# facebookresearch/unbiased-teacher-v2

Hardware: AMD Instinct MI355X
Metric: images/sec/node (labeled+unlabeled) UTv2 step, R50-FPN 1333x800 (higher is better)
Workload: dtype f16

## Files before the change

### include/utv2.h

```cpp
#ifndef UTV2_H
#define UTV2_H
#include <stdint.h>
#ifdef __cplusplus
extern "C" {
#endif

typedef struct ihipStream_t* utv2_stream_t;

int utv2_conv2d_nhwc_fwd(const float* x, const float* w, float* y, const float* scale, const float* bias,
                         const float* residual, int N, int H, int W, int C, int K, int KH, int KW, int stride, int pad,
                         int in_dil, int OH, int OW, int relu, int accumulate, int Kred, utv2_stream_t stream);
int utv2_conv2d_stem_fwd(const float* x, const float* w, void* y, int y_dtype, const float* scale, const float* bias, int N,
                         int H, int W, int K, int KH, int KW, int stride, int pad, int OH, int OW, int relu, int Kred,
                         utv2_stream_t stream);
int utv2_conv2d_wgrad_splits(int N, int OH, int OW, int K, int Kred);
int64_t utv2_conv2d_wgrad_workspace_floats(int N, int OH, int OW, int K, int Kred);
int utv2_conv2d_nhwc_wgrad(const float* x, const float* dy, float* dw, float* ws, int N, int H, int W, int C, int K,
                           int KH, int KW, int stride, int pad, int OH, int OW, int accumulate, utv2_stream_t stream);
int utv2_colsum(const float* g, float* db, float* ws, int M, int C, int accumulate, utv2_stream_t stream);
int utv2_weight_flip_transpose(const float* w, float* wt, int K, int KH, int KW, int C, utv2_stream_t stream);

int utv2_conv2d_ml_fwd(const float* x, const float* w, float* y, const float* scale, const float* bias,
                       const float* residual, int nlev, const int* H_host, const int* W_host, int N, int C, int K, int KH,
                       int KW, int pad, int relu, int accumulate, utv2_stream_t stream);
int utv2_conv2d_ml_wgrad(const float* x, const float* dy, float* dw, float* ws, int nlev, const int* H_host,
                         const int* W_host, int N, int C, int K, int KH, int KW, int pad, int accumulate,
                         utv2_stream_t stream);

#define UTV2_F32 0
#define UTV2_BF16 1
int utv2_conv2d_bf16_supported(int C, int KH, int KW);

int utv2_conv_clock_probe(double* ghz, double* lifetime_us);
int utv2_conv2d_nhwc_fwd_bf16_bits(const void* x, int x_dtype, const void* w16, void* y, int y_dtype, const float* scale,
                                   const float* bias, const void* residual, const void* mask, const void* post_mask, int N, int H, int W,
                                   int C, int K, int KH, int KW, int stride, int pad, int in_dil, int OH, int OW, int relu, int accumulate,
                                   const int* rowinfo, void* relu_bits, const void* mask_bits, const void* post_mask_bits,
                                   utv2_stream_t stream);
int utv2_conv2d_ml_fwd_bf16_g(const void* x, int x_dtype, int x_pitch, const void* w16, void* y, int y_dtype, int y_pitch,
                              const float* scale, const float* bias, const void* residual, int nlev, const int* H_host,
                              const int* W_host, int N, int C, int K, int KH, int KW, int pad, int relu, int accumulate, int groups,
                              float* gn_part, const int* rowinfo, utv2_stream_t stream);
int utv2_conv2d_ml_fwd_bf16_gnb(const void* x, int x_pitch, const void* w16, void* y, int nlev, const int* H_host, const int* W_host, int N,
                                int C, int K, int KH, int KW, int pad, int groups, const int* rowinfo, const void* mask_bits,
                                const void* gnb_x, float* gnb_part, utv2_stream_t stream);
int utv2_conv2d_wgrad_bf16_splits(int M, int K, int Kred);
int64_t utv2_conv2d_wgrad_bf16_workspace_floats(int M, int K, int Kred);
int utv2_conv2d_wgrad_bf16_g(const void* x, int x_dtype, int x_pitch, const void* dy, int dy_dtype, int dy_pitch, float* dw, float* db,
                             float* ws, const int* rowinfo, const float* rowscale, int M, int C, int K, int KH, int KW, int accumulate,
                             int groups, utv2_stream_t stream);
int utv2_conv2d_wgrad_bf16_d(const void* x, int x_dtype, int x_pitch, const void* dy, int dy_dtype, int dy_pitch, float* dw, float* db,
                             float* ws, const int* rowinfo, const float* rowscale, int M, int C, int K, int KH, int KW, int accumulate,
                             int groups, void* pending, utv2_stream_t stream);
int64_t utv2_wgrad_fold_table_bytes(void);
int utv2_wgrad_fold_pending(const void* pending);
int utv2_wgrad_fold_flush(void* pending, utv2_stream_t stream);
int utv2_conv2d_stem_fwd_bf16(const void* xpad16, const void* w16s, void* y, int y_dtype, const float* scale,
                              const float* bias, int N, int H, int W, int K, int OH, int OW, int relu, utv2_stream_t stream);
int utv2_rowinfo_nhwc(int* out, int N, int H, int W, int OH, int OW, int stride, int pad, int KH, int KW, int64_t start,
                      utv2_stream_t stream);
int utv2_f32_to_bf16(const float* src, void* dst16, int64_t n, utv2_stream_t stream);
int utv2_weight_flip_transpose_bf16(const float* w, void* wt16, const float* scale, int K, int KH, int KW, int C,
                                    utv2_stream_t stream);
int utv2_pad_cols_bf16(const void* src, int src_dtype, void* dst16, int64_t rows, int c, int cpad, utv2_stream_t stream);
int utv2_weight_flip_transpose_bf16_batched(const float* arena, const float* scales, void* bank, const void* table, int nlayers,
                                            utv2_stream_t stream);

int utv2_ema_axpby(float* teacher, const float* student, int64_t n, double keep_rate, utv2_stream_t stream);
int utv2_sgd_momentum(float* param, float* grad, float* mom_buf, int64_t n, float lr, float momentum, float weight_decay,
                      float grad_scale, int zero_grad, utv2_stream_t stream);
int utv2_amp_found_inf(const float* grad, int64_t n, float* state, utv2_stream_t stream);
int utv2_sgd_momentum_amp(float* param, const float* grad, float* mom_buf, int64_t n, float lr, float momentum, float weight_decay,
                          float grad_scale, const float* state, utv2_stream_t stream);
int utv2_amp_update_scale(float* state, float growth_factor, float backoff_factor, int growth_interval, utv2_stream_t stream);
int utv2_ema_axpby_m16(float* teacher, const float* student, void* mirror16, int64_t n, double keep_rate, utv2_stream_t stream);
int utv2_sgd_momentum_m16(float* param, float* grad, float* mom_buf, void* mirror16, int64_t n, float lr, float momentum, float weight_decay,
                          float grad_scale, int zero_grad, utv2_stream_t stream);
int utv2_sgd_momentum_amp_m16(float* param, const float* grad, float* mom_buf, void* mirror16, int64_t n, float lr, float momentum,
                              float weight_decay, float grad_scale, const float* state, utv2_stream_t stream);

int utv2_relu_bwd_scale(const void* dy, const void* y, const float* scale, void* out, int64_t M, int C, int dtype,
                        utv2_stream_t stream);
int utv2_add(const float* a, const float* b, float* out, int64_t n, utv2_stream_t stream);
int utv2_maxpool3x3s2_nhwc(const void* x, int x_dtype, void* y, int y_dtype, int N, int H, int W, int C, int OH, int OW,
                           utv2_stream_t stream);
int utv2_maxpool3x3s2_bwd_nhwc(const void* x, int x_dtype, const void* dpool, void* dx, int g_dtype, int N, int H, int W, int C, int OH,
                               int OW, int relu, utv2_stream_t stream);
int utv2_upsample2x_add_nhwc(const void* lateral, const void* top, void* out, int N, int H, int W, int C, int dtype,
                             utv2_stream_t stream);
int utv2_downsample2x_sum_nhwc(const void* g, void* dtop, int N, int TH, int TW, int C, int accumulate, int dtype,
                               utv2_stream_t stream);
int utv2_zero_interleave2x_nhwc(const void* src, const void* mask, void* dst, int N, int H, int W, int C, int dtype, utv2_stream_t stream);
int utv2_zero_interleave2x_add_nhwc(const void* src, const void* mask, const void* mask_bits, const void* add, void* dst, int N, int H, int W,
                                    int C, utv2_stream_t stream);
int utv2_preprocess_image(const void* src, int is_u8, float* dst, int H, int W, int Hp, int Wp,
                          const float* mean3_host, const float* std3_host, utv2_stream_t stream);
int utv2_preprocess_image_bf16pad(const void* src, int is_u8, void* dst16, int H, int W, int Hp, int Wp,
                                  const float* mean3_host, const float* std3_host, utv2_stream_t stream);
int utv2_preprocess_images_bf16pad(const void* const* src_host, int is_u8, void* dst16, const int* H_host, const int* W_host, int N,
                                   int Hp, int Wp, const float* mean3_host, const float* std3_host, utv2_stream_t stream);
int utv2_frozenbn_fold(const float* w, const float* b, const float* mean, const float* var, float* scale, float* shift,
                       int n, float eps, utv2_stream_t stream);
int64_t utv2_groupnorm_seg_workspace_floats(int nseg, const int* seg_rows_host, int C);
int utv2_groupnorm_relu_seg_fwd(const void* x, const float* gamma, const float* beta, void* y, float* mean, float* rstd,
                                float* ws, int nseg, const int* seg_rows_host, int C, int G, float eps, int relu, int dtype,
                                utv2_stream_t stream);
int utv2_groupnorm_relu_seg_fwd_p32(const void* x, const float* gamma, const float* beta, void* y, float* mean, float* rstd,
                                    const float* part32, int nseg, const int* seg_rows_host, int C, int G, float eps, int relu,
                                    utv2_stream_t stream);
int utv2_groupnorm_relu_seg_fwd_p32b(const void* x, const float* gamma, const float* beta, void* y, float* mean, float* rstd,
                                     const float* part32, int nseg, const int* seg_rows_host, int C, int G, float eps, int relu,
                                     void* relu_bits, utv2_stream_t stream);
int utv2_groupnorm_relu_seg_bwd(const void* dy, const void* y, const void* x, const float* mean, const float* rstd,
                                const float* gamma, const float* beta, void* dx, float* dgamma, float* dbeta, float* ws,
                                int nseg, const int* seg_rows_host, int C, int G, int relu, int dtype, utv2_stream_t stream);
int64_t utv2_groupnorm_seg_chunks(int nseg, const int* seg_rows_host);
int utv2_groupnorm_relu_seg_bwd_colsum(const void* dy, const void* y, const void* x, const float* mean, const float* rstd,
                                       const float* gamma, const float* beta, void* dx, float* dgamma, float* dbeta, float* ws,
                                       int nseg, const int* seg_rows_host, int C, int G, int relu, int dtype, float* colsum_part,
                                       utv2_stream_t stream);
int utv2_groupnorm_seg_bwd_p64(const void* g, const void* x, const float* mean, const float* rstd, const float* gamma, void* dx,
                               float* dgamma, float* dbeta, float* ws, int nseg, const int* seg_rows_host, int C, int G,
                               const float* part64, float* colsum_part, utv2_stream_t stream);
int utv2_colsum_partials(const float* partial, float* db, int nb, int K, int accumulate, utv2_stream_t stream);
int64_t utv2_groupnorm_workspace_floats(int N, int HW, int C);
int utv2_groupnorm_relu_fwd(const float* x, const float* gamma, const float* beta, float* y, float* mean, float* rstd,
                            float* ws, int N, int HW, int C, int G, float eps, int relu, utv2_stream_t stream);
int utv2_groupnorm_relu_bwd(const float* dy, const float* y, const float* x, const float* mean, const float* rstd,
                            const float* gamma, float* dx, float* dgamma, float* dbeta, float* ws, int N, int HW, int C,
                            int G, int relu, utv2_stream_t stream);

int utv2_fcos_targets(int num_levels, const int* H_host, const int* W_host, const int* strides_host,
                      const float* soi_host, int N, int MAXG, const float* gt_boxes, const int* gt_classes,
                      const unsigned char* gt_valid, const float* gt_std, int num_classes, int drop_empty,
                      float center_radius, const unsigned char* img_active, int* labels, float* reg_targets, float* bvars,
                      int* gt_inds, utv2_stream_t stream);
int utv2_fcos_targets_range(int num_levels, const int* H_host, const int* W_host, const int* strides_host, const float* soi_host, int N,
                            int MAXG, const float* gt_boxes, const int* gt_classes, const unsigned char* gt_valid, const float* gt_std,
                            int gt_img0, int gt_imgs, int num_classes, int drop_empty, float center_radius,
                            const unsigned char* img_active, int* labels, float* reg_targets, float* bvars, int* gt_inds,
                            utv2_stream_t stream);
int utv2_sigmoid_focal_fwd(const float* logits, const int* labels, int64_t P, int C, float alpha, float gamma,
                           float* loss_sum, float* ws, utv2_stream_t stream);
int utv2_sigmoid_focal_bwd(const float* logits, const int* labels, int64_t P, int C, float alpha, float gamma,
                           const float* coef, float* dlogits, utv2_stream_t stream);
int utv2_fcos_loc_terms_fwd(const int* labels, const float* box, int box_stride, const float* reg_targets,
                            const float* bvars, int64_t P, int num_classes, int reg_max, float ts_better, float ts_cert,
                            int flags, float* sums, float* ws, utv2_stream_t stream);
int utv2_fcos_loc_terms_bwd(const int* labels, const float* box, int box_stride, const float* reg_targets,
                            const float* bvars, int64_t P, int num_classes, int reg_max, float ts_better, float ts_cert,
                            int flags, const float* coef, float* dbox, utv2_stream_t stream);
int utv2_sigmoid_focal_bwd_acc(const float* logits, const int* labels, int64_t P, int C, float alpha, float gamma, const float* coef,
                               const float* gscale, float* dlogits, int accumulate, utv2_stream_t stream);
int utv2_fcos_loc_terms_bwd_acc(const int* labels, const float* box, int box_stride, const float* reg_targets, const float* bvars,
                                int64_t P, int num_classes, int reg_max, float ts_better, float ts_cert, int flags, const float* coef8,
                                const float* gscale, float* dbox, int accumulate, utv2_stream_t stream);
int utv2_fcos_loss_combine(const float* focal_sup, const float* sums_sup, const float* focal_cls, const float* sums_cls,
                           const float* sums_reg, const float* norm, float world, int flags, float kl_weight, const float* wmul_host,
                           const float* wdiv_host, float* rec, float* coef, utv2_stream_t stream);
int utv2_fcos_rank_keys(const float* logits, const float* box, int box_stride, int reg_max, int N, int HW, int C,
                        float thr, int method, long long* keys, int64_t key_row_stride, utv2_stream_t stream);
int64_t utv2_topk_rows_workspace_bytes(int rows, int k);
int utv2_topk_rows_i64(const long long* keys, const long long* row_off, int rows, int64_t max_width, int k, long long* out,
                       void* ws, utv2_stream_t stream);
int utv2_fcos_decode(const long long* topkeys, int K, const float* logits, const float* box, int box_stride, int reg_max,
                     int N, int HW, int Wl, int C, int stride, int level, int method, int MAXC, int slot0, float* oboxes,
                     float* oscores, int* ocls, float* oloc, float* octr, float* oconf, float* ostd, int* olevel,
                     unsigned char* ovalid, utv2_stream_t stream);
int utv2_fcos_loc_terms_cont_fwd(const int* labels, const float* box, int box_stride, const float* reg_targets, const float* bvars,
                                 int64_t P, int num_classes, float ts_better, float ts_cert, int flags, float* sums, float* ws,
                                 utv2_stream_t stream);
int utv2_fcos_loc_terms_cont_bwd(const int* labels, const float* box, int box_stride, const float* reg_targets, const float* bvars,
                                 int64_t P, int num_classes, float ts_better, float ts_cert, int flags, const float* coef, float* dbox,
                                 utv2_stream_t stream);
int utv2_fcos_loc_terms_cont_bwd_acc(const int* labels, const float* box, int box_stride, const float* reg_targets, const float* bvars,
                                     int64_t P, int num_classes, float ts_better, float ts_cert, int flags, const float* coef8,
                                     const float* gscale, float* dbox, int accumulate, utv2_stream_t stream);
int utv2_fcos_decode_cont(const long long* topkeys, int K, const float* logits, const float* box, int box_stride, int N, int HW, int Wl,
                          int C, int stride, int level, int method, int MAXC, int slot0, float* oboxes, float* oscores, int* ocls,
                          float* oloc, float* octr, float* oconf, float* ostd, int* olevel, unsigned char* ovalid,
                          utv2_stream_t stream);
int utv2_scale_cols(float* y, int64_t rows, int row_stride, int ncols, const float* s, utv2_stream_t stream);
int utv2_scale_cols_bwd(float* g, const float* ypost, int64_t rows, int row_stride, int ncols, const float* s, float* dsum,
                        float* ws, utv2_stream_t stream);
int utv2_scale_cols_ml(float* y, int nlev, const int64_t* row0_host, int row_stride, int ncols, const float* const* s_host,
                       utv2_stream_t stream);
int utv2_scale_cols_bwd_ml(float* g, const float* ypost, int nlev, const int64_t* row0_host, int row_stride, int ncols,
                           const float* const* s_host, float* const* sgrad_host, float* ws, utv2_stream_t stream);
int utv2_scale_cols_bwd_ml_pad16(const float* g, const float* ypost, int nlev, const int64_t* row0_host, int row_stride, int ncols,
                                 const float* const* s_host, float* const* sgrad_host, float* ws, void* out16, int cpad, utv2_stream_t stream);

int utv2_nms_mpad(int M);
int64_t utv2_nms_workspace_bytes(int N, int M);
int utv2_nms_batched(const float* boxes, const float* scores, const int* cls, const unsigned char* valid, int N, int M,
                     float iou_thr, int class_aware, int post_topk, int max_out, int* keep, int* keep_count, void* ws,
                     utv2_stream_t stream);
int utv2_box_iou(const float* a, const float* b, int A, int B, float* out, utv2_stream_t stream);

int utv2_match_boxes(const float* boxes, int64_t box_img_stride, int N, int P, const float* gt_boxes,
                     const unsigned char* gt_valid, int G, float* max_iou, int* arg, unsigned* gt_max_bits,
                     utv2_stream_t stream);
int utv2_match_lowq(const float* boxes, int64_t box_img_stride, int N, int P, const float* gt_boxes,
                    const unsigned char* gt_valid, int G, const unsigned* gt_max_bits, unsigned char* lowq,
                    utv2_stream_t stream);
#define UTV2_POOLER_ALIGN_V2 0
#define UTV2_POOLER_ALIGN 1
#define UTV2_POOLER_MAX 2
int utv2_roi_pooler_fwd(int pooler, int sampling_ratio, int num_levels, int min_level, const void* const* feats_host,
                        const int* H_host, const int* W_host, const float* scales_host, const float* rois, const int* roi_batch,
                        const unsigned char* roi_valid, int R, int C, int PH, int PW, void* out, int* argmax, int dtype,
                        utv2_stream_t stream);
int utv2_roi_pooler_bwd(int pooler, int sampling_ratio, int num_levels, int min_level, float* const* dfeats_host, const int* H_host,
                        const int* W_host, const float* scales_host, const float* rois, const int* roi_batch,
                        const unsigned char* roi_valid, int R, int C, int PH, int PW, const void* dy, const int* argmax, int dtype,
                        utv2_stream_t stream);
int utv2_roi_pooler_bwd_tiled(int pooler, int sampling_ratio, int num_levels, int min_level, void* const* dfeats_host,
                              const int* H_host, const int* W_host, const float* scales_host, const float* rois,
                              const unsigned char* roi_valid, int N, int rois_per_image, int C, int PH, int PW, const void* dy,
                              const int* argmax, int dy_dtype, int out_dtype, utv2_stream_t stream);
int utv2_rpn_rank_keys(const float* head, int num_levels, const int* hw_host, int N, int A, int ch, int64_t* keys, utv2_stream_t stream);
int utv2_rpn_decode(const int64_t* top, int maxk, const float* head, const float* anchors, const float* image_hw, int num_levels,
                    const int* hw_host, const int* k_host, int N, int A, int ch, const float* weights_host, float scale_clamp,
                    float min_size, float* boxes, float* scores, int* lvls, unsigned char* keep, utv2_stream_t stream);
int utv2_nms_pack(const int* kidx, const int* cnt, const float* boxes, const float* scores, int N, int M, int D, float* oboxes, float* oscores,
                  unsigned char* ovalid, utv2_stream_t stream);
int utv2_roi_infer_keys(const float* probs, const float* deltas, const float* prop, const unsigned char* valid, const float* whwh, int N, int P,
                        int K, int nbox, float wx, float wy, float scale_clamp, float thr, float* boxes, int64_t* keys, utv2_stream_t stream);
int utv2_roi_infer_gather(const int64_t* top, const float* boxes, int N, int P, int K, int nbox, int k, float thr, float* sc, int64_t* rows,
                          int* cls, float* cb, unsigned char* valid, utv2_stream_t stream);
int utv2_roi_infer_pack(const int* kidx, const int* cnt, const float* cb, const float* sc, const int* cls, const int64_t* rows, const float* stdl,
                        int N, int P, int k, int D, int nbox, float* oboxes, float* oscores, int* ocls, float* ostd, int64_t* orows,
                        unsigned char* ovalid, utv2_stream_t stream);
int utv2_rpn_loss_fwd(const float* obj, const float* deltas, int head, int num_levels, const int* hw_host, int N, int A, int ch, int R,
                      const float* anchors, const int64_t* pos_idx, const unsigned char* pos_valid, int npos, const int64_t* neg_idx,
                      const unsigned char* neg_valid, int nneg, const int* matched, const unsigned char* has_gt, const float* gt_boxes,
                      const float* gt_scores, int G, const float* weights_host, float* sums, float* gobj, float* gdl, utv2_stream_t stream);
int utv2_rpn_loss_bwd(const float* gobj, const float* gdl, const float* gout_cls, const float* gout_loc, int head, int num_levels,
                      const int* hw_host, int N, int A, int ch, int R, const int64_t* pos_idx, const unsigned char* pos_valid, int npos,
                      const int64_t* neg_idx, const unsigned char* neg_valid, int nneg, float* grad_obj, float* grad_deltas,
                      utv2_stream_t stream);
int utv2_rpn_loss_fwd_range(const float* obj, const float* deltas, int head, int num_levels, const int* hw_host, int N, int batch, int img0,
                            int A, int ch, int R, const float* anchors, const int64_t* pos_idx, const unsigned char* pos_valid, int npos,
                            const int64_t* neg_idx, const unsigned char* neg_valid, int nneg, const int* matched,
                            const unsigned char* has_gt, const float* gt_boxes, const float* gt_scores, int G, const float* weights_host,
                            float* sums, float* gobj, float* gdl, utv2_stream_t stream);
int utv2_rpn_loss_bwd_range(const float* gobj, const float* gdl, const float* gout_cls, const float* gout_loc, int head, int num_levels,
                            const int* hw_host, int N, int batch, int img0, int A, int ch, int R, const int64_t* pos_idx,
                            const unsigned char* pos_valid, int npos, const int64_t* neg_idx, const unsigned char* neg_valid, int nneg,
                            float* grad_obj, float* grad_deltas, utv2_stream_t stream);
int utv2_rpn_sample_keys(const float* max_iou, const unsigned char* lowq, const unsigned char* gt_valid, int G, const float* keys, int N,
                         int R, float lo, float hi, int64_t* out, utv2_stream_t stream);
int utv2_rpn_sample_unpack(const int64_t* top, int k, int N, int npos_max, int nneg_max, const unsigned char* gt_valid, int G,
                           int64_t* pos_idx, unsigned char* pos_valid, int64_t* neg_idx, unsigned char* neg_valid, unsigned char* has_gt,
                           utv2_stream_t stream);
int utv2_roi_sample(const float* boxes, const unsigned char* valid, const float* max_iou, const int* argmax, const float* keys, int N, int P,
                    const float* gt_boxes, const int* gt_classes, const unsigned char* gt_valid, const float* gt_scores, const float* gt_std,
                    int G, float iou_thr, int num_classes, int batch, int nfg_max, float* out_boxes, int64_t* out_classes,
                    float* out_gt_boxes, unsigned char* out_valid, int64_t* out_idx, float* out_conf, float* out_std, utv2_stream_t stream);
int utv2_roi_box_loss(const float* deltas, const float* stdl, int64_t ld, const int64_t* cls, const float* prop, const float* gtb,
                      const float* gstd, int R, int num_classes, int nbox, int mode, float wx, float wy, float scale_clamp, float ts_better,
                      float t_cert, float* sum, float* gdeltas, float* gstd_out, utv2_stream_t stream);
int utv2_softmax_focal_fwd(const float* logits, const int* target, int R, int C, float gamma, float* loss_sum, float* ws,
                           utv2_stream_t stream);
int utv2_softmax_focal_bwd(const float* logits, const int* target, int R, int C, float gamma, const float* coef,
                           float* dlogits, utv2_stream_t stream);
int utv2_rcnn_loss_combine(const float* rpn_sup, const float* rpn_uns, const float* focal_sup, const float* focal_uns, const float* box_sup,
                           const float* box_uns, const int* tgt_sup, int n_sup, const int* tgt_uns, int n_uns, float rpn_norm_sup,
                           float rpn_norm_uns, float w_rpn_cls, float w_rpn_loc, float w_box, const float* wt_host, float* rec, float* coef,
                           utv2_stream_t stream);

int utv2_stem_pool_fwd_bf16(const void* xpad16, const void* w16s, void* y, const float* scale, const float* shift, int N, int H, int W,
                            int K, utv2_stream_t stream);

int utv2_bottleneck_supported(int C, int MID, int has_shortcut);
int utv2_bottleneck_fwd_bf16(const void* x, void* y, const void* w1, const void* w2, const void* w3, const void* wsc, const float* s1,
                             const float* b1, const float* s2, const float* b2, const float* s3, const float* b3, const float* ssc,
                             const float* bsc, int N, int H, int W, int C, int MID, utv2_stream_t stream);

int64_t utv2_aug_resize_workspace_bytes(int H, int W, int OH, int OW);
int utv2_aug_resize_bilinear_u8(const unsigned char* src, int H, int W, unsigned char* dst, int OH, int OW, int flip, void* ws,
                                utv2_stream_t stream);
int utv2_aug_gray_mean_u8(const unsigned char* img, int64_t npix, void* sum_ws, int* mean_out, utv2_stream_t stream);
int utv2_aug_blend_u8(unsigned char* img, int64_t npix, int mode, float alpha, const int* mean, utv2_stream_t stream);
int utv2_aug_hue_u8(unsigned char* img, int64_t npix, int shift, utv2_stream_t stream);
int utv2_aug_grayscale_u8(unsigned char* img, int64_t npix, utv2_stream_t stream);
int utv2_aug_box_blur_u8(const unsigned char* src, unsigned char* dst, int H, int W, int vertical, int radius, int ww, int fw,
                         utv2_stream_t stream);
int utv2_aug_erase_u8(unsigned char* img, int H, int W, int i, int j, int h, int w, const float* noise, utv2_stream_t stream);
int utv2_aug_hwc_to_chw_u8(const unsigned char* src, unsigned char* dst, int64_t npix, utv2_stream_t stream);

int utv2_coco_pair_keys(const float* scores, const int* cls, const long long* off, int N, int K, long long* keys, utv2_stream_t stream);
int utv2_coco_seg_offsets(const long long* keys, int64_t n, int64_t nseg, long long* off, utv2_stream_t stream);
int utv2_coco_rank_keys(const long long* key1, const long long* pair_off, int64_t D, int K, int max_dets, long long* key2,
                        unsigned char* rank, utv2_stream_t stream);
int64_t utv2_coco_eval_workspace_bytes(int64_t D, int K);
int utv2_coco_match(const float* dbox, const long long* dperm, const long long* dpair_off, const double* gbox, const unsigned char* gcrowd,
                    const double* garea, const long long* gperm, const long long* gpair_off, int N, int K, int64_t D, int max_dets,
                    int max_gt, const double* iou_thrs_host, const double* area_rng_host, void* ws, utv2_stream_t stream);
int utv2_coco_accumulate(const long long* perm2, const long long* cat_off, const unsigned char* rank, int K, int64_t D,
                         const double* rec_thrs_host, const void* ws, double* precision, double* recall, utv2_stream_t stream);

int utv2_gconv3x3_supported(int C, int G);
int utv2_gconv3x3_fwd(const void* x, const void* w, int op_dtype, void* y, int y_dtype, const float* scale, const float* shift, int N,
                      int H, int W, int C, int G, int stride, int OH, int OW, int relu, utv2_stream_t stream);
int utv2_gconv3x3_dgrad(const void* dy, const void* w, int op_dtype, void* dx, int dx_dtype, const float* scale, const void* mask,
                        const void* residual, int N, int H, int W, int C, int G, int stride, int OH, int OW, utv2_stream_t stream);
int utv2_gconv3x3_wgrad_splits(int N, int OH, int OW, int C, int G);
int64_t utv2_gconv3x3_wgrad_workspace_floats(int N, int OH, int OW, int C, int G);
int utv2_gconv3x3_wgrad(const void* x, const void* dy, int op_dtype, float* dw, float* ws, const float* scale, int N, int H, int W,
// ... 7 lines not shown
```

### unbiased-teacher-v2_amd/csrc/fcos.hip

```cpp
#include "common.h"

#define MAX_LEVELS 8

struct LevelTable {
  int num_levels;
  int H[MAX_LEVELS], W[MAX_LEVELS], stride[MAX_LEVELS];
  int off[MAX_LEVELS + 1];
  float soi_lo[MAX_LEVELS], soi_hi[MAX_LEVELS];
};

__device__ __forceinline__ int level_of(const LevelTable& t, int loc) {
  int l = 0;
#pragma unroll
  for (int i = 1; i < MAX_LEVELS; ++i)
    if (i < t.num_levels && loc >= t.off[i]) l = i;
  return l;
}

#define TG_MAXG 256
__global__ __launch_bounds__(256) void fcos_targets_kernel(LevelTable lt, int N, int MAXG, const float* __restrict__ gt_boxes,
                                                         const int* __restrict__ gt_classes,
                                                         const unsigned char* __restrict__ gt_valid,
                                                         const float* __restrict__ gt_std, int num_classes, int drop_empty,
                                                         float center_radius, const unsigned char* __restrict__ img_active,
// ... 19 lines not shown
  const int G = scount;
  for (int k = threadIdx.x; k < G; k += blockDim.x) {
    const float* b = gt_boxes + ((size_t)gi * MAXG + sidx[k]) * 4;
    sb[k][0] = b[0]; sb[k][1] = b[1]; sb[k][2] = b[2]; sb[k][3] = b[3];
    sarea[k] = (b[2] - b[0]) * (b[3] - b[1]);
  }
  __syncthreads();
  const int loc = blockIdx.x * blockDim.x + threadIdx.x;
  if (loc >= L) return;
  const int l = level_of(lt, loc);
  const int hw = loc - lt.off[l];
  const int HWl = lt.H[l] * lt.W[l];
  const int y = hw / lt.W[l], x = hw - y * lt.W[l];
  const float s = (float)lt.stride[l];
  const float xs = (float)(x * lt.stride[l]) + (float)(lt.stride[l] / 2);
  const float ys = (float)(y * lt.stride[l]) + (float)(lt.stride[l] / 2);
  const size_t p = (size_t)N * lt.off[l] + (size_t)n * HWl + hw;
  const bool inactive = !in_range || (img_active != nullptr && !img_active[n]);
  if (G == 0 || inactive) {
    labels[p] = ((drop_empty & 1) || inactive) ? -1 : num_classes;
    gt_inds[p] = -1;
#pragma unroll
    for (int e = 0; e < 4; ++e) { reg_targets[p * 4 + e] = 0.f; bvars[p * 4 + e] = 0.f; }
    return;
  }
  const float INF = 100000000.f;
  float best = INF;
  int bi = 0;
  const bool cs = center_radius > 0.f;
  const float sr = s * center_radius;
  const bool cs_none = cs && (sb[0][0] + sb[0][2]) * 0.5f * (float)L == 0.f;
  bool inside_any = false, sampled_any = false;
  for (int k = 0; k < G; ++k) {
    const float lft = xs - sb[k][0], top = ys - sb[k][1], rgt = sb[k][2] - xs, bot = sb[k][3] - ys;
    float mn = fminf(fminf(lft, top), fminf(rgt, bot));
    inside_any |= mn > 0.f;
    const float mx = fmaxf(fmaxf(lft, top), fmaxf(rgt, bot));
    if (cs) {
      const float cx = (sb[k][0] + sb[k][2]) * 0.5f, cy = (sb[k][1] + sb[k][3]) * 0.5f;
      const float xmin = cx - sr, ymin = cy - sr, xmax = cx + sr, ymax = cy + sr;
      const float x0 = xmin > sb[k][0] ? xmin : sb[k][0], y0 = ymin > sb[k][1] ? ymin : sb[k][1];
      const float x1 = xmax > sb[k][2] ? sb[k][2] : xmax, y1 = ymax > sb[k][3] ? sb[k][3] : ymax;
      mn = cs_none ? -1.f : fminf(fminf(xs - x0, ys - y0), fminf(x1 - xs, y1 - ys));
    }
    sampled_any |= mn > 0.f;
    float a = sarea[k];
    if (!(mn > 0.f)) a = INF;
    if (!(mx >= lt.soi_lo[l] && mx <= lt.soi_hi[l])) a = INF;
    if (a < best) { best = a; bi = k; }
  }
  const bool bg = (best == INF);
  const int g = sidx[bi];
  const bool ignored = (drop_empty & 2) && inside_any && !sampled_any;
  labels[p] = ignored ? -1 : bg ? num_classes : gt_classes[gi * MAXG + g];
  gt_inds[p] = g;
  reg_targets[p * 4 + 0] = (xs - sb[bi][0]) / s;
  reg_targets[p * 4 + 1] = (ys - sb[bi][1]) / s;
  reg_targets[p * 4 + 2] = (sb[bi][2] - xs) / s;
  reg_targets[p * 4 + 3] = (sb[bi][3] - ys) / s;
#pragma unroll
  for (int e = 0; e < 4; ++e) bvars[p * 4 + e] = bg ? 99999.0f : (gt_std ? gt_std[((size_t)gi * MAXG + g) * 4 + e] : 0.f);
}

__device__ __forceinline__ float focal_term(float x, float t, float alpha, float gamma, float* dldx) {
  const float e = expf(-fabsf(x));
  const float r = 1.f / (1.f + e);
  const float p = x >= 0.f ? r : e * r;
  const float l1p = log1pf(e);
  const float ce = fmaxf(x, 0.f) - x * t + l1p;
  const float q = x >= 0.f ? e * r : r;
  const float pt = p * t + q * (1.f - t);
  const float om = q * t + p * (1.f - t);
  const float mod = (gamma == 2.f) ? om * om : powf(om, gamma);
  const float at = alpha >= 0.f ? alpha * t + (1.f - alpha) * (1.f - t) : 1.f;
  if (dldx) {
    *dldx = at * (2.f * t - 1.f) * mod * (gamma * pt * (-ce) - om);
  }
  return ce * mod * at;
}

__global__ __launch_bounds__(256) void focal_fwd_kernel(const float* __restrict__ logits, const int* __restrict__ labels, size_t P,
                                                      int C, float alpha, float gamma, float* __restrict__ partial) {
  __shared__ float red[4];
  float acc = 0.f;
  if ((C & 3) == 0 && P * (size_t)C < (1ull << 32)) {
    const unsigned C4 = (unsigned)C >> 2, total4 = (unsigned)(P * (size_t)C4);
    for (unsigned i4 = blockIdx.x * blockDim.x + threadIdx.x; i4 < total4; i4 += gridDim.x * blockDim.x) {
      const unsigned row = i4 / C4;
      const int c = (int)(i4 - row * C4) * 4;
      const int lab = labels[row];
      if (lab < 0) continue;
      const f32x4 v = ((const f32x4*)logits)[i4];
#pragma unroll
      for (int e = 0; e < 4; ++e) acc += focal_term(v[e], lab == c + e ? 1.f : 0.f, alpha, gamma, nullptr);
    }
  } else {
    const size_t total = P * (size_t)C;
    const size_t stride = (size_t)gridDim.x * blockDim.x;
    for (size_t i = (size_t)blockIdx.x * blockDim.x + threadIdx.x; i < total; i += stride) {
      const size_t row = i / C;
      const int c = (int)(i - row * C);
      const int lab = labels[row];
      if (lab < 0) continue;
      acc += focal_term(logits[i], lab == c ? 1.f : 0.f, alpha, gamma, nullptr);
    }
  }
  const float s = block_reduce_sum(acc, red);
  if (threadIdx.x == 0) partial[blockIdx.x] = s;
}

__global__ __launch_bounds__(256) void focal_bwd_kernel(const float* __restrict__ logits, const int* __restrict__ labels, size_t P,
                                                      int C, float alpha, float gamma, const float* __restrict__ coef,
                                                      float* __restrict__ dlogits, const float* __restrict__ gscale, int accumulate) {
  const float k = coef[0] * (gscale ? gscale[0] : 1.f);
  if ((C & 3) == 0 && P * (size_t)C < (1ull << 32)) {
    const unsigned C4 = (unsigned)C >> 2, total4 = (unsigned)(P * (size_t)C4);
    for (unsigned i4 = blockIdx.x * blockDim.x + threadIdx.x; i4 < total4; i4 += gridDim.x * blockDim.x) {
      const unsigned row = i4 / C4;
      const int c = (int)(i4 - row * C4) * 4;
      const int lab = labels[row];
      if (accumulate && lab < 0) continue;
      f32x4 g = {0.f, 0.f, 0.f, 0.f};
      if (accumulate) g = ((const f32x4*)dlogits)[i4];
      if (lab >= 0) {
        const f32x4 v = ((const f32x4*)logits)[i4];
#pragma unroll
        for (int e = 0; e < 4; ++e) {
          float ge;
          focal_term(v[e], lab == c + e ? 1.f : 0.f, alpha, gamma, &ge);
          g[e] += ge * k;
        }
      }
      ((f32x4*)dlogits)[i4] = g;
    }
    return;
  }
  const size_t total = P * (size_t)C;
  size_t i = (size_t)blockIdx.x * blockDim.x + threadIdx.x;
  const size_t stride = (size_t)gridDim.x * blockDim.x;
  for (; i < total; i += stride) {
    const size_t row = i / C;
    const int c = (int)(i - row * C);
    const int lab = labels[row];
    if (accumulate && lab < 0) continue;
    float g = 0.f;
    if (lab >= 0) {
      focal_term(logits[i], lab == c ? 1.f : 0.f, alpha, gamma, &g);
      g *= k;
    }
    dlogits[i] = accumulate ? dlogits[i] + g : g;
  }
}

__global__ __launch_bounds__(256) void sum_partials_kernel(const float* __restrict__ partial, int n, int ncols,
                                                           float* __restrict__ out) {
  __shared__ double red[256];
  const int c = blockIdx.x;
  double s = 0.0;
  for (int r = threadIdx.x; r < n; r += 256) s += (double)partial[(size_t)r * ncols + c];
  red[threadIdx.x] = s;
  __syncthreads();
  for (int w = 128; w > 0; w >>= 1) {
    if (threadIdx.x < w) red[threadIdx.x] += red[threadIdx.x + w];
    __syncthreads();
  }
  if (threadIdx.x == 0) out[c] = (float)red[0];
}

#define LT_NSUM 8
struct LocTerms {
  float d[4];
  float ctr_t, iou, giou_l, nll;
};

template <int R1>
__device__ __forceinline__ void integral4(const float* __restrict__ z, float* d, float (*prob)[R1]) {
#pragma unroll
  for (int b = 0; b < 4; ++b) {
    float m = -INFINITY;
#pragma unroll
    for (int j = 0; j < R1; ++j) m = fmaxf(m, z[b * R1 + j]);
    int jm = 0;
#pragma unroll
    for (int j = R1 - 1; j >= 0; --j)
      if (z[b * R1 + j] == m) jm = j;
    float s = 0.f, e[R1];
#pragma unroll
    for (int j = 0; j < R1; ++j) { e[j] = expf(z[b * R1 + j] - m); s += e[j]; }
    float acc = 0.f;
#pragma unroll
    for (int j = 0; j < R1; ++j) {
      const float pj = e[j] / s;
      if (prob) prob[b][j] = pj;
      acc += pj * (float)(j - jm);
    }
    d[b] = (float)jm + acc;
  }
}

__device__ __forceinline__ float min_grad(float a, float b) { return a < b ? 1.f : (a == b ? 0.5f : 0.f); }
__device__ __forceinline__ float max_grad(float a, float b) { return a > b ? 1.f : (a == b ? 0.5f : 0.f); }

__device__ __forceinline__ float giou_ltrb(const float* d, const float* t, float* iou_out, float* grad, int loc_type = 0) {
  const float ta = (t[0] + t[2]) * (t[1] + t[3]);
  const float pw = d[0] + d[2], ph = d[1] + d[3];
  const float pa = pw * ph;
  const float wi = fminf(d[0], t[0]) + fminf(d[2], t[2]);
  const float hi = fminf(d[3], t[3]) + fminf(d[1], t[1]);
  const float gw = fmaxf(d[0], t[0]) + fmaxf(d[2], t[2]);
  const float gh = fmaxf(d[3], t[3]) + fmaxf(d[1], t[1]);
  const float ac = gw * gh;
  const float I = wi * hi;
  const float U = ta + pa - I;
  const float iou = (I + 1.f) / (U + 1.f);
  const float giou = iou - (ac - U) / ac;
  if (iou_out) *iou_out = iou;
  if (grad) {
#pragma unroll
    for (int b = 0; b < 4; ++b) {
      const bool horiz = (b == 0 || b == 2);
      const float dpa = horiz ? ph : pw;
      const float dI = horiz ? min_grad(d[b], t[b]) * hi : min_grad(d[b], t[b]) * wi;
      const float dac = horiz ? max_grad(d[b], t[b]) * gh : max_grad(d[b], t[b]) * gw;
      const float dU = dpa - dI;
      const float diou = (dI * (U + 1.f) - (I + 1.f) * dU) / ((U + 1.f) * (U + 1.f));
      const float dgiou = diou + dU / ac - U * dac / (ac * ac);
      float g = -diou;
      if (loc_type == 1) g = g / iou;
      if (loc_type == 0) g = -dgiou;
      grad[b] = g;
    }
  }
  return loc_type == 0 ? 1.f - giou : (loc_type == 1 ? -logf(iou) : 1.f - iou);
}

__device__ __forceinline__ double min_grad_f64(double a, double b) { return a < b ? 1.0 : (a == b ? 0.5 : 0.0); }
__device__ __forceinline__ double max_grad_f64(double a, double b) { return a > b ? 1.0 : (a == b ? 0.5 : 0.0); }
__device__ __forceinline__ double giou_ltrb_f64(const double* d, const double* t, double* iou_out, double* grad, int loc_type) {
  const double ta = (t[0] + t[2]) * (t[1] + t[3]);
  const double pw = d[0] + d[2], ph = d[1] + d[3];
  const double pa = pw * ph;
  const double wi = fmin(d[0], t[0]) + fmin(d[2], t[2]);
  const double hi = fmin(d[3], t[3]) + fmin(d[1], t[1]);
  const double gw = fmax(d[0], t[0]) + fmax(d[2], t[2]);
  const double gh = fmax(d[3], t[3]) + fmax(d[1], t[1]);
  const double ac = gw * gh;
  const double I = wi * hi;
  const double U = ta + pa - I;
  const double iou = (I + 1.0) / (U + 1.0);
  const double giou = iou - (ac - U) / ac;
  if (iou_out) *iou_out = iou;
  if (grad) {
#pragma unroll
    for (int b = 0; b < 4; ++b) {
      const bool horiz = (b == 0 || b == 2);
      const double dpa = horiz ? ph : pw;
      const double dI = horiz ? min_grad_f64(d[b], t[b]) * hi : min_grad_f64(d[b], t[b]) * wi;
      const double dac = horiz ? max_grad_f64(d[b], t[b]) * gh : max_grad_f64(d[b], t[b]) * gw;
      const double dU = dpa - dI;
      const double diou = (dI * (U + 1.0) - (I + 1.0) * dU) / ((U + 1.0) * (U + 1.0));
      const double dgiou = diou + dU / ac - U * dac / (ac * ac);
      double g = -diou;
      if (loc_type == 1) g = g / iou;
      if (loc_type == 0) g = -dgiou;
      grad[b] = g;
    }
  }
  return loc_type == 0 ? 1.0 - giou : (loc_type == 1 ? -log(iou) : 1.0 - iou);
}

#define LT_QUALITY_IOU 1
#define LT_KLLOSS 2
#define LT_LOC_SHIFT 2
#define LT_KL_WCTR 16

template <int R1>
__global__ __launch_bounds__(128) void fcos_loc_fwd_kernel(const int* __restrict__ labels, const float* __restrict__ box, int BS,
                                                         const float* __restrict__ reg_targets, const float* __restrict__ bvars,
                                                         size_t P, int num_classes, float ts_better, float ts_cert, int flags,
                                                         float* __restrict__ partial) {
  __shared__ float red[2];
  float acc[LT_NSUM];
#pragma unroll
  for (int k = 0; k < LT_NSUM; ++k) acc[k] = 0.f;
  size_t i = (size_t)blockIdx.x * blockDim.x + threadIdx.x;
  const size_t stride = (size_t)gridDim.x * blockDim.x;
  for (; i < P; i += stride) {
    const int lab = labels[i];
    if (lab < 0 || lab == num_classes) continue;
    const float* row = box + i * BS;
    float d[4], t[4];
    integral4<R1>(row, d, (float(*)[R1]) nullptr);
#pragma unroll
    for (int b = 0; b < 4; ++b) t[b] = reg_targets[i * 4 + b];
    float ctr_t = sqrtf((fminf(t[0], t[2]) / fmaxf(t[0], t[2])) * (fminf(t[1], t[3]) / fmaxf(t[1], t[3])));
    float iou;
    const float gl = giou_ltrb(d, t, &iou, nullptr, (flags >> LT_LOC_SHIFT) & 3);
    if (flags & LT_QUALITY_IOU) ctr_t = iou;
    float nll = 0.f;
    const float* sp = row + 4 * R1;
    if (flags & LT_KLLOSS) {
#pragma unroll
      for (int b = 0; b < 4; ++b) {
        const float n = fabsf(d[b] - t[b]);
        nll += expf(-sp[b]) * (n < 1.f ? 0.5f * n * n : n - 0.5f) + 0.5f * sp[b];
      }
      iou = (flags & LT_KL_WCTR) ? ctr_t : 1.f;
    } else {
#pragma unroll
      for (int b = 0; b < 4; ++b) {
        const float sg = 1.f / (1.f + expf(-sp[b]));
        const float sq = sg * sg;
        const float df = t[b] - d[b];
        nll += (df * df) / (2.f * sq) + 0.5f * logf(sq);
      }
      nll += 2.f * logf(2.f * 3.14159265358979323846f);
    }
    const float c = row[4 * R1 + 4];
    const float bce = fmaxf(c, 0.f) - c * ctr_t + log1pf(expf(-fabsf(c)));
    acc[0] += 1.f;
    acc[1] += ctr_t;
    acc[2] += bce;
    acc[3] += gl * ctr_t;
    acc[4] += nll * iou;
    if (bvars) {
#pragma unroll
      for (int b = 0; b < 4; ++b) {
        const float cs = 1.f - 1.f / (1.f + expf(-sp[b]));
        const float ct = 1.f - 1.f / (1.f + expf(-bvars[i * 4 + b]));
        if (ct > ts_cert && ct > cs + ts_better) {
          acc[5] += 1.f;
          acc[6] += fabsf(d[b] - t[b]);
        }
      }
    }
  }
#pragma unroll
  for (int k = 0; k < LT_NSUM; ++k) {
    const float s = block_reduce_sum(acc[k], red);
    if (threadIdx.x == 0) partial[(size_t)blockIdx.x * LT_NSUM + k] = s;
  }
}

template <int R1>
__global__ __launch_bounds__(128) void fcos_loc_bwd_kernel(const int* __restrict__ labels, const float* __restrict__ box, int BS,
                                                         const float* __restrict__ reg_targets, const float* __restrict__ bvars,
                                                         size_t P, int num_classes, float ts_better, float ts_cert, int flags,
                                                         const float* __restrict__ coef, float* __restrict__ dbox,
                                                         const float* __restrict__ gscale, int coef8, int accumulate) {
  size_t i = (size_t)blockIdx.x * blockDim.x + threadIdx.x;
  const size_t stride = (size_t)gridDim.x * blockDim.x;
  const float gs = gscale ? gscale[0] : 1.f;
  const float c_bce = coef[coef8 ? 2 : 0] * gs, c_giou = coef[coef8 ? 3 : 1] * gs, c_nll = coef[coef8 ? 4 : 2] * gs,
              c_l1 = coef[coef8 ? 6 : 3] * gs;
  for (; i < P; i += stride) {
    const int lab = labels[i];
    float* grow = dbox + i * BS;
    if (lab < 0 || lab == num_classes) {
      if (!accumulate)
        for (int k = 0; k < BS; k += 4) *(f32x4*)(grow + k) = f32x4{0.f, 0.f, 0.f, 0.f};
      continue;
    }
    const float* row = box + i * BS;
    double d[4], t[4], dl[4], prob[4][R1];
    int jm[4];
#pragma unroll
    for (int b = 0; b < 4; ++b) {
      float m = -INFINITY;
#pragma unroll
      for (int j = 0; j < R1; ++j) m = fmaxf(m, row[b * R1 + j]);
      int q = 0;
#pragma unroll
      for (int j = R1 - 1; j >= 0; --j)
        if (row[b * R1 + j] == m) q = j;
      double s = 0.0;
#pragma unroll
      for (int j = 0; j < R1; ++j) { prob[b][j] = exp((double)row[b * R1 + j] - (double)m); s += prob[b][j]; }
      double acc = 0.0;
#pragma unroll
      for (int j = 0; j < R1; ++j) { prob[b][j] /= s; acc += prob[b][j] * (double)(j - q); }
      jm[b] = q; dl[b] = acc; d[b] = (double)q + acc;
      t[b] = (double)reg_targets[i * 4 + b];
    }
    double ctr_t = sqrt((fmin(t[0], t[2]) / fmax(t[0], t[2])) * (fmin(t[1], t[3]) / fmax(t[1], t[3])));
    double iou, gg[4];
    giou_ltrb_f64(d, t, &iou, gg, (flags >> LT_LOC_SHIFT) & 3);
    if (flags & LT_QUALITY_IOU) ctr_t = iou;
    const float* sp = row + 4 * R1;
    double dd[4], ds[4];
#pragma unroll
    for (int b = 0; b < 4; ++b) {
      const double sg = 1.0 / (1.0 + exp(-(double)sp[b]));
      const double df = d[b] == t[b] ? 0.0 : (t[b] - (double)jm[b]) - dl[b];
      if (flags & LT_KLLOSS) {
        const double n = fabs(df), es = exp(-(double)sp[b]);
        const double sgn = df < 0.0 ? 1.0 : (df > 0.0 ? -1.0 : 0.0);
        const double wk = (flags & LT_KL_WCTR) ? ctr_t : 1.0;
        dd[b] = (double)c_giou * ctr_t * gg[b] + (double)c_nll * wk * es * fmin(n, 1.0) * sgn;
        ds[b] = (double)c_nll * wk * (0.5 - es * (n < 1.0 ? 0.5 * n * n : n - 0.5));
      } else {
        dd[b] = (double)c_giou * ctr_t * gg[b] + (double)c_nll * iou * (-df / (sg * sg));
        ds[b] = (double)c_nll * iou * (1.0 - sg) * (1.0 - (df * df) / (sg * sg));
      }
      if (bvars) {
        const float cs = 1.f - 1.f / (1.f + expf(-sp[b]));
        const float ct = 1.f - 1.f / (1.f + expf(-bvars[i * 4 + b]));
        if (ct > ts_cert && ct > cs + ts_better) dd[b] += (double)c_l1 * (d[b] > t[b] ? 1.0 : (d[b] < t[b] ? -1.0 : 0.0));
      }
    }
    const double c = (double)row[4 * R1 + 4];
    const float dctr = (float)((double)c_bce * (1.0 / (1.0 + exp(-c)) - ctr_t));
    if (accumulate) {
#pragma unroll
      for (int b = 0; b < 4; ++b)
#pragma unroll
        for (int j = 0; j < R1; ++j) grow[b * R1 + j] += (float)(dd[b] * prob[b][j] * ((double)(j - jm[b]) - dl[b]));
#pragma unroll
      for (int b = 0; b < 4; ++b) grow[4 * R1 + b] += (float)ds[b];
      grow[4 * R1 + 4] += dctr;
      continue;
    }
#pragma unroll
    for (int b = 0; b < 4; ++b)
#pragma unroll
      for (int j = 0; j < R1; ++j) grow[b * R1 + j] = (float)(dd[b] * prob[b][j] * ((double)(j - jm[b]) - dl[b]));
#pragma unroll
    for (int b = 0; b < 4; ++b) grow[4 * R1 + b] = (float)ds[b];
    grow[4 * R1 + 4] = dctr;
    for (int k = 4 * R1 + 5; k < BS; ++k) grow[k] = 0.f;
  }
}

__global__ __launch_bounds__(256) void fcos_rank_keys_kernel(const float* __restrict__ logits, const float* __restrict__ box, int BS,
                                                           int R4, int HW, int C, float thr, int method,
                                                           long long* __restrict__ keys, size_t key_stride) {
  const int n = blockIdx.y;
  const size_t total = (size_t)HW * C;
  size_t i = (size_t)blockIdx.x * blockDim.x + threadIdx.x;
  const size_t stride = (size_t)gridDim.x * blockDim.x;
  for (; i < total; i += stride) {
    const size_t hw = i / C;
    const size_t row = (size_t)n * HW + hw;
    const float p = 1.f / (1.f + expf(-logits[row * C + (i - hw * C)]));
    long long key = -1;
    if (p > thr) {
      float r = p;
      const float* br = box + row * BS;
      if (method == 1) r = p * (1.f / (1.f + expf(-br[R4 + 4])));
      else if (method == 2) r = 1.f / (1.f + expf(-br[R4 + 4]));
      else if (method == 3) {
        float m = 0.f;
#pragma unroll
        for (int b = 0; b < 4; ++b) m += 1.f - 1.f / (1.f + expf(-br[R4 + b]));
        r = p * (m / 4.f);
      }
      key = ((long long)__float_as_uint(r) << 32) | (long long)(0xFFFFFFFFu - (unsigned)i);
    }
    keys[(size_t)n * key_stride + i] = key;
  }
}

template <int R1>
__global__ __launch_bounds__(128) void fcos_decode_kernel(const long long* __restrict__ topkeys, int K, const float* __restrict__ logits,
                                                        const float* __restrict__ box, int BS, int HW, int Wl, int C, int stride,
                                                        int level, int method, int MAXC, int slot0, float* __restrict__ oboxes,
                                                        float* __restrict__ oscores, int* __restrict__ ocls, float* __restrict__ oloc,
                                                        float* __restrict__ octr, float* __restrict__ oconf, float* __restrict__ ostd,
                                                        int* __restrict__ olevel, unsigned char* __restrict__ ovalid) {
  const int n = blockIdx.y;
  const int k = blockIdx.x * blockDim.x + threadIdx.x;
  if (k >= K) return;
  const size_t s = (size_t)n * MAXC + slot0 + k;
  const long long key = topkeys[(size_t)n * K + k];
  if (key < 0) {
    ovalid[s] = 0;
    oscores[s] = -1.f;
    ocls[s] = 0;
    olevel[s] = level;
#pragma unroll
    for (int e = 0; e < 4; ++e) { oboxes[s * 4 + e] = 0.f; ostd[s * 4 + e] = 0.f; }
    oloc[s * 2] = 0.f; oloc[s * 2 + 1] = 0.f; octr[s] = 0.f; oconf[s] = 0.f;
    return;
  }
  const unsigned flat = 0xFFFFFFFFu - (unsigned)(key & 0xFFFFFFFFll);
  const float rank = __uint_as_float((unsigned)(key >> 32));
  const int hw = flat / C, c = flat - hw * C;
  const size_t row = (size_t)n * HW + hw;
  const float* br = box + row * BS;
  float d[4];
  integral4<R1>(br, d, (float(*)[R1]) nullptr);
  const int y = hw / Wl, x = hw - y * Wl;
  const float lx = (float)(x * stride) + (float)(stride / 2), ly = (float)(y * stride) + (float)(stride / 2);
  const float fs = (float)stride;
  oboxes[s * 4 + 0] = lx - d[0] * fs;
  oboxes[s * 4 + 1] = ly - d[1] * fs;
  oboxes[s * 4 + 2] = lx + d[2] * fs;
  oboxes[s * 4 + 3] = ly + d[3] * fs;
  oscores[s] = (method == 1 || method == 3) ? sqrtf(rank) : rank;
  ocls[s] = c;
  oloc[s * 2] = lx; oloc[s * 2 + 1] = ly;
  octr[s] = 1.f / (1.f + expf(-br[4 * R1 + 4]));
  oconf[s] = 1.f / (1.f + expf(-logits[row * C + c]));
#pragma unroll
  for (int e = 0; e < 4; ++e) ostd[s * 4 + e] = br[4 * R1 + e];
  olevel[s] = level;
  ovalid[s] = 1;
}

#define CT_STD 4
#define CT_CTR 8
#define CT_COLS 9

__global__ __launch_bounds__(128) void fcos_loc_cont_fwd_kernel(const int* __restrict__ labels, const float* __restrict__ box, int BS,
                                                              const float* __restrict__ reg_targets, const float* __restrict__ bvars,
                                                              size_t P, int num_classes, float ts_better, float ts_cert, int flags,
                                                              float* __restrict__ partial) {
  __shared__ float red[2];
  float acc[LT_NSUM];
#pragma unroll
  for (int k = 0; k < LT_NSUM; ++k) acc[k] = 0.f;
  size_t i = (size_t)blockIdx.x * blockDim.x + threadIdx.x;
  const size_t stride = (size_t)gridDim.x * blockDim.x;
  for (; i < P; i += stride) {
    const int lab = labels[i];
    if (lab < 0 || lab == num_classes) continue;
    const float* row = box + i * BS;
    float d[4], t[4];
#pragma unroll
    for (int b = 0; b < 4; ++b) { d[b] = fmaxf(row[b], 0.f); t[b] = reg_targets[i * 4 + b]; }
    float ctr_t = sqrtf((fminf(t[0], t[2]) / fmaxf(t[0], t[2])) * (fminf(t[1], t[3]) / fmaxf(t[1], t[3])));
    float iou;
    const float gl = giou_ltrb(d, t, &iou, nullptr, (flags >> LT_LOC_SHIFT) & 3);
    if (flags & LT_QUALITY_IOU) ctr_t = iou;
    float nll = 0.f;
    const float* sp = row + CT_STD;
    if (flags & LT_KLLOSS) {
#pragma unroll
      for (int b = 0; b < 4; ++b) {
        const float n = fabsf(d[b] - t[b]);
        nll += expf(-sp[b]) * (n < 1.f ? 0.5f * n * n : n - 0.5f) + 0.5f * sp[b];
      }
      iou = (flags & LT_KL_WCTR) ? ctr_t : 1.f;
    } else {
#pragma unroll
      for (int b = 0; b < 4; ++b) {
        const float sg = 1.f / (1.f + expf(-sp[b]));
        const float sq = sg * sg;
        const float df = t[b] - d[b];
        nll += (df * df) / (2.f * sq) + 0.5f * logf(sq);
      }
      nll += 2.f * logf(2.f * 3.14159265358979323846f);
    }
    const float c = row[CT_CTR];
    const float bce = fmaxf(c, 0.f) - c * ctr_t + log1pf(expf(-fabsf(c)));
    acc[0] += 1.f;
    acc[1] += ctr_t;
    acc[2] += bce;
    acc[3] += gl * ctr_t;
    acc[4] += nll * iou;
    if (bvars) {
#pragma unroll
      for (int b = 0; b < 4; ++b) {
        const float cs = 1.f - 1.f / (1.f + expf(-sp[b]));
        const float ct = 1.f - 1.f / (1.f + expf(-bvars[i * 4 + b]));
        if (ct > ts_cert && ct > cs + ts_better) {
          acc[5] += 1.f;
          acc[6] += fabsf(d[b] - t[b]);
        }
      }
    }
  }
#pragma unroll
  for (int k = 0; k < LT_NSUM; ++k) {
    const float s = block_reduce_sum(acc[k], red);
    if (threadIdx.x == 0) partial[(size_t)blockIdx.x * LT_NSUM + k] = s;
  }
}

__global__ __launch_bounds__(128) void fcos_loc_cont_bwd_kernel(const int* __restrict__ labels, const float* __restrict__ box, int BS,
                                                              const float* __restrict__ reg_targets, const float* __restrict__ bvars,
                                                              size_t P, int num_classes, float ts_better, float ts_cert, int flags,
                                                              const float* __restrict__ coef, float* __restrict__ dbox,
// ... 231 lines not shown
  for (int l = 0; l < MAX_LEVELS; ++l) {
    if (l < num_levels) {
      t.H[l] = H[l]; t.W[l] = W[l]; t.stride[l] = strides[l];
      t.soi_lo[l] = soi ? soi[2 * l] : 0.f; t.soi_hi[l] = soi ? soi[2 * l + 1] : 0.f;
      t.off[l] = off;
      off += H[l] * W[l];
    } else {
      t.H[l] = t.W[l] = t.stride[l] = 0; t.soi_lo[l] = t.soi_hi[l] = 0.f; t.off[l] = off;
    }
  }
  t.off[num_levels] = off;
  for (int l = num_levels + 1; l <= MAX_LEVELS; ++l) t.off[l] = off;
  return t;
}

struct FcosCombineArgs {
  const float* focal_sup;
  const float* sums_sup;
  const float* focal_cls;
  const float* sums_cls;
  const float* sums_reg;
  const float* norm;
  float world, kl_weight;
  int flags;
  float wmul[6], wdiv[6];
};

__global__ void fcos_loss_combine_kernel(FcosCombineArgs a, float* __restrict__ rec, float* __restrict__ coef) {
  if (threadIdx.x != 0 || blockIdx.x != 0) return;
  for (int i = 0; i < 26; ++i) coef[i] = 0.f;
  const bool kl = a.flags & 1, kl4 = a.flags & 2, unify = a.flags & 4, tsb = a.flags & 8;
  float g[6];
  for (int k = 0; k < 6; ++k) g[k] = a.wmul[k] / a.wdiv[k];
  const float* S = a.sums_sup;
  const float npa_s = fmaxf((a.norm ? a.norm[0] : S[0]) / a.world, 1.f), den_s = fmaxf((a.norm ? a.norm[1] : S[1]) / a.world, 1e-6f);
  const float cls = a.focal_sup[0] / npa_s, ctr = S[2] / npa_s;
  float loc = S[3] / den_s;
  coef[0] = g[0] / npa_s;
  coef[1 + 2] = g[2] / npa_s;
  coef[1 + 3] = g[1] / den_s;
  if (kl) {
    const float n = fmaxf(S[0], 1.f), dn = kl4 ? 4.f * n : n, w = a.kl_weight;
    loc = w * (w * (S[4] / dn)) + loc;
    coef[1 + 4] = g[1] * (w * w) / dn;
  }
  const float* C = a.sums_cls;
  const float npa_c = fmaxf((a.norm ? a.norm[2] : C[0]) / a.world, 1.f);
  const float cls_p = a.focal_cls[0] / npa_c;
  float ctr_p = C[2] / npa_c;
  coef[9] = g[3] / npa_c;
  if (unify) ctr_p = ctr_p * 0.f;
  else coef[10 + 2] = g[4] / npa_c;
  const float* R = a.sums_reg;
  float loc_p, tbs = 0.f;
  if (tsb) {
    const float d = fmaxf(R[5], 1.f);
    loc_p = R[6] / d;
    tbs = R[5];
    coef[18 + 6] = g[5] / d;
  } else {
    const float n = fmaxf(R[0], 1.f), dn = kl4 ? 4.f * n : n;
    loc_p = a.kl_weight * (R[4] / dn);
    coef[18 + 4] = g[5] * a.kl_weight / dn;
  }
  rec[0] = cls; rec[1] = loc; rec[2] = ctr; rec[3] = cls_p; rec[4] = ctr_p; rec[5] = loc_p; rec[6] = tbs;
  const float v[6] = {cls, loc, ctr, cls_p, ctr_p, loc_p};
  float total = 0.f;
  for (int k = 0; k < 6; ++k) total += v[k] * a.wmul[k] / a.wdiv[k];
  rec[7] = total;
}

extern "C" {

int utv2_fcos_targets_range(int num_levels, const int* H, const int* W, const int* strides, const float* soi, int N, int MAXG,
                            const float* gt_boxes, const int* gt_classes, const unsigned char* gt_valid, const float* gt_std,
                            int gt_img0, int gt_imgs, int num_classes, int drop_empty, float center_radius,
                            const unsigned char* img_active, int* labels, float* reg_targets, float* bvars, int* gt_inds,
                            hipStream_t stream) {
  if (num_levels < 1 || num_levels > MAX_LEVELS || MAXG > TG_MAXG || MAXG < 1 || !gt_boxes || !gt_classes || !gt_valid ||
      !labels || !reg_targets || !bvars || !gt_inds || gt_img0 < 0 || gt_imgs < 0 || gt_img0 + gt_imgs > N)
    return UTV2_EARG;
  LevelTable t = make_table(num_levels, H, W, strides, soi);
  const int L = t.off[num_levels];
  hipLaunchKernelGGL(fcos_targets_kernel, dim3(cdiv(L, 256), N), dim3(256), 0, stream, t, N, MAXG, gt_boxes, gt_classes,
                     gt_valid, gt_std, num_classes, drop_empty, center_radius, img_active, gt_img0, gt_imgs, labels, reg_targets, bvars,
                     gt_inds);
  return utv2_launch_status();
}

int utv2_fcos_targets(int num_levels, const int* H, const int* W, const int* strides, const float* soi, int N, int MAXG,
                      const float* gt_boxes, const int* gt_classes, const unsigned char* gt_valid, const float* gt_std,
                      int num_classes, int drop_empty, float center_radius, const unsigned char* img_active, int* labels,
                      float* reg_targets, float* bvars, int* gt_inds, hipStream_t stream) {
  return utv2_fcos_targets_range(num_levels, H, W, strides, soi, N, MAXG, gt_boxes, gt_classes, gt_valid, gt_std, 0, N, num_classes,
                                 drop_empty, center_radius, img_active, labels, reg_targets, bvars, gt_inds, stream);
}

#define FOCAL_BLOCKS 1024
int utv2_sigmoid_focal_fwd(const float* logits, const int* labels, int64_t P, int C, float alpha, float gamma,
                           float* loss_sum, float* ws, hipStream_t stream) {
  if (!logits || !labels || !loss_sum || !ws || P < 0 || C < 1) return UTV2_EARG;
  hipLaunchKernelGGL(focal_fwd_kernel, dim3(FOCAL_BLOCKS), dim3(256), 0, stream, logits, labels, (size_t)P, C, alpha, gamma, ws);
  hipLaunchKernelGGL(sum_partials_kernel, dim3(1), dim3(256), 0, stream, (const float*)ws, FOCAL_BLOCKS, 1, loss_sum);
  return utv2_launch_status();
}

int utv2_sigmoid_focal_bwd(const float* logits, const int* labels, int64_t P, int C, float alpha, float gamma,
                           const float* coef, float* dlogits, hipStream_t stream) {
  if (!logits || !labels || !coef || !dlogits || P < 0 || C < 1) return UTV2_EARG;
  hipLaunchKernelGGL(focal_bwd_kernel, dim3(2048), dim3(256), 0, stream, logits, labels, (size_t)P, C, alpha, gamma, coef, dlogits,
                     (const float*)nullptr, 0);
  return utv2_launch_status();
}

int utv2_sigmoid_focal_bwd_acc(const float* logits, const int* labels, int64_t P, int C, float alpha, float gamma, const float* coef,
                               const float* gscale, float* dlogits, int accumulate, hipStream_t stream) {
  if (!logits || !labels || !coef || !dlogits || P < 0 || C < 1) return UTV2_EARG;
  hipLaunchKernelGGL(focal_bwd_kernel, dim3(2048), dim3(256), 0, stream, logits, labels, (size_t)P, C, alpha, gamma, coef, dlogits, gscale,
                     accumulate ? 1 : 0);
  return utv2_launch_status();
}

#define LOC_BLOCKS 512
int utv2_fcos_loc_terms_fwd(const int* labels, const float* box, int box_stride, const float* reg_targets,
                            const float* bvars, int64_t P, int num_classes, int reg_max, float ts_better, float ts_cert,
                            int flags, float* sums, float* ws, hipStream_t stream) {
  if (!labels || !box || !reg_targets || !sums || !ws || reg_max != 16 || flags < 0 || ((flags >> LT_LOC_SHIFT) & 3) > 2 || flags >= 32 || box_stride < 4 * 17 + 5 || (box_stride & 3) || P < 0) return UTV2_EARG;
  hipLaunchKernelGGL((fcos_loc_fwd_kernel<17>), dim3(LOC_BLOCKS), dim3(128), 0, stream, labels, box, box_stride, reg_targets,
                     bvars, (size_t)P, num_classes, ts_better, ts_cert, flags, ws);
  hipLaunchKernelGGL(sum_partials_kernel, dim3(LT_NSUM), dim3(256), 0, stream, (const float*)ws, LOC_BLOCKS, LT_NSUM, sums);
  return utv2_launch_status();
}

int utv2_fcos_loc_terms_bwd(const int* labels, const float* box, int box_stride, const float* reg_targets,
                            const float* bvars, int64_t P, int num_classes, int reg_max, float ts_better, float ts_cert,
                            int flags, const float* coef, float* dbox, hipStream_t stream) {
  if (!labels || !box || !reg_targets || !coef || !dbox || reg_max != 16 || flags < 0 || ((flags >> LT_LOC_SHIFT) & 3) > 2 || flags >= 32 || box_stride < 4 * 17 + 5 || (box_stride & 3) || P < 0) return UTV2_EARG;
  if (P == 0) return UTV2_OK;
  hipLaunchKernelGGL((fcos_loc_bwd_kernel<17>), dim3(cdiv(P, 128)), dim3(128), 0, stream, labels, box, box_stride, reg_targets,
                     bvars, (size_t)P, num_classes, ts_better, ts_cert, flags, coef, dbox, (const float*)nullptr, 0, 0);
  return utv2_launch_status();
}

int utv2_fcos_loc_terms_bwd_acc(const int* labels, const float* box, int box_stride, const float* reg_targets, const float* bvars,
                                int64_t P, int num_classes, int reg_max, float ts_better, float ts_cert, int flags, const float* coef8,
                                const float* gscale, float* dbox, int accumulate, hipStream_t stream) {
  if (!labels || !box || !reg_targets || !coef8 || !dbox || reg_max != 16 || flags < 0 || ((flags >> LT_LOC_SHIFT) & 3) > 2 || flags >= 32 || box_stride < 4 * 17 + 5 || (box_stride & 3) || P < 0) return UTV2_EARG;
  if (P == 0) return UTV2_OK;
  hipLaunchKernelGGL((fcos_loc_bwd_kernel<17>), dim3(cdiv(P, 128)), dim3(128), 0, stream, labels, box, box_stride, reg_targets,
                     bvars, (size_t)P, num_classes, ts_better, ts_cert, flags, coef8, dbox, gscale, 1, accumulate ? 1 : 0);
  return utv2_launch_status();
}

int utv2_fcos_rank_keys(const float* logits, const float* box, int box_stride, int reg_max, int N, int HW, int C, float thr,
                        int method, long long* keys, int64_t key_row_stride, hipStream_t stream) {
  if (!logits || !box || !keys || method < 0 || method > 3 || key_row_stride < (int64_t)HW * C) return UTV2_EARG;
  int gx = cdiv((int64_t)HW * C, 256);
  if (gx > 4096) gx = 4096;
  hipLaunchKernelGGL(fcos_rank_keys_kernel, dim3(gx, N), dim3(256), 0, stream, logits, box, box_stride, 4 * (reg_max + 1), HW, C,
                     thr, method, keys, (size_t)key_row_stride);
  return utv2_launch_status();
}

int utv2_fcos_decode(const long long* topkeys, int K, const float* logits, const float* box, int box_stride, int reg_max,
                     int N, int HW, int Wl, int C, int stride, int level, int method, int MAXC, int slot0, float* oboxes,
                     float* oscores, int* ocls, float* oloc, float* octr, float* oconf, float* ostd, int* olevel,
                     unsigned char* ovalid, hipStream_t stream) {
  if (!topkeys || !logits || !box || reg_max != 16 || slot0 + K > MAXC) return UTV2_EARG;
  hipLaunchKernelGGL((fcos_decode_kernel<17>), dim3(cdiv(K, 128), N), dim3(128), 0, stream, topkeys, K, logits, box, box_stride,
                     HW, Wl, C, stride, level, method, MAXC, slot0, oboxes, oscores, ocls, oloc, octr, oconf, ostd, olevel,
                     ovalid);
  return utv2_launch_status();
}

static bool loc_cont_args_bad(const void* labels, const void* box, int box_stride, const void* reg_targets, int64_t P, int flags) {
  return !labels || !box || !reg_targets || flags < 0 || flags >= 32 || ((flags >> LT_LOC_SHIFT) & 3) > 2 || box_stride < CT_COLS ||
         (box_stride & 3) || P < 0;
}

int utv2_fcos_loc_terms_cont_fwd(const int* labels, const float* box, int box_stride, const float* reg_targets, const float* bvars,
                                 int64_t P, int num_classes, float ts_better, float ts_cert, int flags, float* sums, float* ws,
                                 hipStream_t stream) {
  if (loc_cont_args_bad(labels, box, box_stride, reg_targets, P, flags) || !sums || !ws) return UTV2_EARG;
  int nb = (int)(P < (int64_t)LOC_BLOCKS * 128 ? cdiv(P, 128) : LOC_BLOCKS);
  if (nb < 1) nb = 1;
  hipLaunchKernelGGL(fcos_loc_cont_fwd_kernel, dim3(nb), dim3(128), 0, stream, labels, box, box_stride, reg_targets, bvars, (size_t)P,
                     num_classes, ts_better, ts_cert, flags, ws);
  hipLaunchKernelGGL(sum_partials_kernel, dim3(LT_NSUM), dim3(256), 0, stream, (const float*)ws, nb, LT_NSUM, sums);
  return utv2_launch_status();
}

int utv2_fcos_loc_terms_cont_bwd(const int* labels, const float* box, int box_stride, const float* reg_targets, const float* bvars,
                                 int64_t P, int num_classes, float ts_better, float ts_cert, int flags, const float* coef, float* dbox,
                                 hipStream_t stream) {
  if (loc_cont_args_bad(labels, box, box_stride, reg_targets, P, flags) || !coef || !dbox || cdiv(P, 128) > 0x7fffffffll) return UTV2_EARG;
  if (P == 0) return UTV2_OK;
  hipLaunchKernelGGL(fcos_loc_cont_bwd_kernel, dim3((unsigned)cdiv(P, 128)), dim3(128), 0, stream, labels, box, box_stride, reg_targets,
                     bvars, (size_t)P, num_classes, ts_better, ts_cert, flags, coef, dbox, (const float*)nullptr, 0, 0);
  return utv2_launch_status();
}

int utv2_fcos_loc_terms_cont_bwd_acc(const int* labels, const float* box, int box_stride, const float* reg_targets, const float* bvars,
                                     int64_t P, int num_classes, float ts_better, float ts_cert, int flags, const float* coef8,
                                     const float* gscale, float* dbox, int accumulate, hipStream_t stream) {
  if (loc_cont_args_bad(labels, box, box_stride, reg_targets, P, flags) || !coef8 || !dbox || cdiv(P, 128) > 0x7fffffffll) return UTV2_EARG;
  if (P == 0) return UTV2_OK;
  hipLaunchKernelGGL(fcos_loc_cont_bwd_kernel, dim3((unsigned)cdiv(P, 128)), dim3(128), 0, stream, labels, box, box_stride, reg_targets,
                     bvars, (size_t)P, num_classes, ts_better, ts_cert, flags, coef8, dbox, gscale, 1, accumulate ? 1 : 0);
  return utv2_launch_status();
}

int utv2_fcos_decode_cont(const long long* topkeys, int K, const float* logits, const float* box, int box_stride, int N, int HW, int Wl,
                          int C, int stride, int level, int method, int MAXC, int slot0, float* oboxes, float* oscores, int* ocls,
                          float* oloc, float* octr, float* oconf, float* ostd, int* olevel, unsigned char* ovalid, hipStream_t stream) {
  if (!topkeys || !logits || !box || !oboxes || !oscores || !ocls || !oloc || !octr || !oconf || !ostd || !olevel || !ovalid ||
      box_stride < CT_COLS || (box_stride & 3) || K < 0 || N < 1 || N > 65535 || HW < 1 || Wl < 1 || Wl > HW || C < 1 || stride < 1 ||
      method < 0 || method > 3 || slot0 < 0 || MAXC < 0 || (int64_t)slot0 + K > MAXC || (int64_t)HW * C > 0xFFFFFFFFll)
    return UTV2_EARG;
  if (K == 0) return UTV2_OK;
  hipLaunchKernelGGL(fcos_decode_cont_kernel, dim3(cdiv(K, 128), N), dim3(128), 0, stream, topkeys, K, logits, box, box_stride, HW, Wl, C,
                     stride, level, method, MAXC, slot0, oboxes, oscores, ocls, oloc, octr, oconf, ostd, olevel, ovalid);
  return utv2_launch_status();
}

int utv2_scale_cols(float* y, int64_t rows, int row_stride, int ncols, const float* s, hipStream_t stream) {
  if (!y || !s) return UTV2_EARG;
  int g = cdiv(rows * ncols, 256);
  if (g > 4096) g = 4096;
  hipLaunchKernelGGL(scale_cols_kernel, dim3(g), dim3(256), 0, stream, y, (size_t)rows, row_stride, ncols, s);
  return utv2_launch_status();
}

int utv2_scale_cols_bwd(float* g, const float* ypost, int64_t rows, int row_stride, int ncols, const float* s, float* dsum,
                        float* ws, hipStream_t stream) {
  if (!g || !ypost || !s || !dsum || !ws) return UTV2_EARG;
  int nb = cdiv(rows * ncols, 256);
  if (nb > 1024) nb = 1024;
  hipLaunchKernelGGL(scale_cols_bwd_kernel, dim3(nb), dim3(256), 0, stream, g, ypost, (size_t)rows, row_stride, ncols, s, ws);
  hipLaunchKernelGGL(sum_partials_kernel, dim3(1), dim3(256), 0, stream, (const float*)ws, nb, 1, dsum);
  return utv2_launch_status();
}

static int fill_scale_levels(ScaleLevels& L, int nlev, const int64_t* row0_host, const float* const* s_host, float* const* sgrad_host) {
  if (nlev < 1 || nlev > SC_MAXL || !row0_host || !s_host) return UTV2_EARG;
  L.nlev = nlev;
  for (int l = 0; l <= SC_MAXL; ++l) L.row0[l] = row0_host[l <= nlev ? l : nlev];
  for (int l = 0; l < SC_MAXL; ++l) {
    L.s[l] = l < nlev ? s_host[l] : nullptr;
    L.sgrad[l] = (l < nlev && sgrad_host) ? sgrad_host[l] : nullptr;
    if (l < nlev && (!L.s[l] || L.row0[l + 1] < L.row0[l])) return UTV2_EARG;
  }
  return UTV2_OK;
}

int utv2_scale_cols_ml(float* y, int nlev, const int64_t* row0_host, int row_stride, int ncols, const float* const* s_host,
                       hipStream_t stream) {
  ScaleLevels L;
  if (!y || fill_scale_levels(L, nlev, row0_host, s_host, nullptr) != UTV2_OK) return UTV2_EARG;
  int64_t most = 0;
  for (int l = 0; l < nlev; ++l) most = L.row0[l + 1] - L.row0[l] > most ? L.row0[l + 1] - L.row0[l] : most;
  int gx = cdiv(most * ncols, 256 * 4);
  if (gx > 1024) gx = 1024;
  if (gx < 1) gx = 1;
  hipLaunchKernelGGL(scale_cols_ml_kernel, dim3(gx, nlev), dim3(256), 0, stream, y, L, row_stride, ncols);
  return utv2_launch_status();
}

int utv2_scale_cols_bwd_ml(float* g, const float* ypost, int nlev, const int64_t* row0_host, int row_stride, int ncols,
                           const float* const* s_host, float* const* sgrad_host, float* ws, hipStream_t stream) {
  ScaleLevels L;
  if (!g || !ypost || !ws || !sgrad_host || fill_scale_levels(L, nlev, row0_host, s_host, sgrad_host) != UTV2_OK) return UTV2_EARG;
  for (int l = 0; l < nlev; ++l)
    if (!L.sgrad[l]) return UTV2_EARG;
  const int nb = 1024;
  int64_t rows_max = 0;
  for (int l = 0; l < nlev; ++l) rows_max = rows_max > row0_host[l + 1] - row0_host[l] ? rows_max : row0_host[l + 1] - row0_host[l];
  const bool vec4 = (row_stride & 3) == 0 && (ncols & 3) == 0 && (((uintptr_t)g | (uintptr_t)ypost) & 15) == 0 &&
                    rows_max * (row_stride >> 2) < (int64_t)1 << 31;
  if (vec4) hipLaunchKernelGGL(scale_cols_bwd_ml_kernel<true>, dim3(nb, nlev), dim3(256), 0, stream, g, ypost, L, row_stride, ncols, ws);
  else hipLaunchKernelGGL(scale_cols_bwd_ml_kernel<false>, dim3(nb, nlev), dim3(256), 0, stream, g, ypost, L, row_stride, ncols, ws);
  hipLaunchKernelGGL(scale_cols_bwd_ml_final, dim3(nlev), dim3(256), 0, stream, L, (const float*)ws, nb);
  return utv2_launch_status();
}

int utv2_scale_cols_bwd_ml_pad16(const float* g, const float* ypost, int nlev, const int64_t* row0_host, int row_stride, int ncols,
                                 const float* const* s_host, float* const* sgrad_host, float* ws, void* out16, int cpad, hipStream_t stream) {
  ScaleLevels L;
  if (!g || !ypost || !ws || !sgrad_host || !out16 || fill_scale_levels(L, nlev, row0_host, s_host, sgrad_host) != UTV2_OK) return UTV2_EARG;
  for (int l = 0; l < nlev; ++l)
    if (!L.sgrad[l]) return UTV2_EARG;
  int64_t rows_max = 0;
  for (int l = 0; l < nlev; ++l) rows_max = rows_max > row0_host[l + 1] - row0_host[l] ? rows_max : row0_host[l + 1] - row0_host[l];
  if ((row_stride & 3) || (ncols & 3) || (cpad & 3) || cpad < row_stride || ncols > row_stride || ((((uintptr_t)g | (uintptr_t)ypost) & 15) != 0) ||
      (((uintptr_t)out16) & 7) != 0 || rows_max * (cpad >> 2) >= (int64_t)1 << 31)
    return UTV2_EARG;
  const int nb = 1024;
  hipLaunchKernelGGL(scale_cols_bwd_ml_pad16_kernel, dim3(nb, nlev), dim3(256), 0, stream, g, ypost, L, row_stride, ncols, ws, (h16_t*)out16, cpad);
  hipLaunchKernelGGL(scale_cols_bwd_ml_final, dim3(nlev), dim3(256), 0, stream, L, (const float*)ws, nb);
  return utv2_launch_status();
}

int utv2_fcos_loss_combine(const float* focal_sup, const float* sums_sup, const float* focal_cls, const float* sums_cls,
                           const float* sums_reg, const float* norm, float world, int flags, float kl_weight, const float* wmul_host,
                           const float* wdiv_host, float* rec, float* coef, hipStream_t stream) {
  if (!focal_sup || !sums_sup || !focal_cls || !sums_cls || !sums_reg || !wmul_host || !wdiv_host || !rec || !coef || !(world >= 1.f))
    return UTV2_EARG;
// ... 10 lines not shown
```

### unbiased-teacher-v2_amd/ubteacher/hip.py

```python
import ctypes
import os

import torch

_HERE = os.path.dirname(os.path.abspath(__file__))
_LIB_DIR = os.environ.get("UTV2_LIB_DIR") or os.path.join(os.path.dirname(_HERE), "lib")
LIB_PATH = os.path.join(_LIB_DIR, "libutv2_hip.so")
LIB_PATHS = {"bf16": LIB_PATH, "fp16": os.path.join(_LIB_DIR, "libutv2_hip_f16.so")}
H16 = ["bf16"]


_H16_DT = [torch.bfloat16]


def set_h16(kind):
    assert kind in LIB_PATHS
    H16[0] = kind
    _H16_DT[0] = torch.bfloat16 if kind == "bf16" else torch.float16


def h16_dtype():
    return _H16_DT[0]

_lib = None
# ... 334 lines not shown
            out = torch.zeros((len(images), Hm + 6, Wm + 8, 4), dtype=h16_dtype(), device=dev)
            _stem_in_cache[key] = out
        n = len(images)
        dt = images[0].dtype
        if n <= 32 and all(im.dtype == dt for im in images):
            for im in images:
                assert im.is_cuda and im.is_contiguous() and im.dtype in (torch.uint8, torch.float32)
            ptrs = (ctypes.c_void_p * n)(*[im.data_ptr() for im in images])
            call("utv2_preprocess_images_bf16pad", ctypes.cast(ptrs, c_p), int(dt == torch.uint8), _p(out), ctypes.cast(_iarr([a for a, _ in sizes]), c_p),
                 ctypes.cast(_iarr([b for _, b in sizes]), c_p), n, Hm, Wm, ctypes.cast(m, c_p), ctypes.cast(s, c_p), _stream())
        else:
            for i, im in enumerate(images):
                assert im.is_contiguous() and im.dtype in (torch.uint8, torch.float32)
                call("utv2_preprocess_image_bf16pad", _p(im), int(im.dtype == torch.uint8), c_p(out[i].data_ptr()), sizes[i][0],
                     sizes[i][1], Hm, Wm, ctypes.cast(m, c_p), ctypes.cast(s, c_p), _stream())
        out.canvas = (Hm, Wm)
        return out, sizes
    out = torch.empty((len(images), Hm, Wm, 4), dtype=torch.float32, device=dev)
    for i, im in enumerate(images):
        assert im.is_contiguous() and im.dtype in (torch.uint8, torch.float32)
        call("utv2_preprocess_image", _p(im), int(im.dtype == torch.uint8), c_p(out[i].data_ptr()), sizes[i][0],
             sizes[i][1], Hm, Wm, ctypes.cast(m, c_p), ctypes.cast(s, c_p), _stream())
    return out, sizes


def conv2d_stem_fwd_bf16(xpad16, w16s, scale, bias, relu, out_dtype):
    N = xpad16.shape[0]
    H, W = xpad16.canvas
    K = w16s.shape[0]
    OH, OW = conv_out_size(H, 7, 2, 3), conv_out_size(W, 7, 2, 3)
    out = torch.empty((N, OH, OW, K), dtype=out_dtype, device=xpad16.device)
    call("utv2_conv2d_stem_fwd_bf16", _p(xpad16), _p(w16s), _p(out), _dt(out), _p(scale), _p(bias), N, H, W, K, OH, OW,
         int(relu), _stream())
    return out


def stem_pool_fwd_bf16(xpad16, w16s, scale, shift):
    N = xpad16.shape[0]
    H, W = xpad16.canvas
    K = w16s.shape[0]
    OH, OW = conv_out_size(H, 7, 2, 3), conv_out_size(W, 7, 2, 3)
    PH, PW = (OH + 2 - 3) // 2 + 1, (OW + 2 - 3) // 2 + 1
    out = torch.empty((N, PH, PW, K), dtype=h16_dtype(), device=xpad16.device)
    call("utv2_stem_pool_fwd_bf16", _p(xpad16), _p(w16s), _p(out), _p(scale), _p(shift), N, H, W, K, _stream())
    return out


def stem_weight_image(w208):
    K = w208.shape[0]
    w = w208[:, :196].reshape(K, 7, 28)
    return torch.nn.functional.pad(w, (0, 4)).reshape(K, 224).to(h16_dtype()).contiguous()


def frozenbn_fold(w, b, mean, var, scale, shift, eps=1e-5):
    call("utv2_frozenbn_fold", _p(w), _p(b), _p(mean), _p(var), _p(scale), _p(shift), w.numel(), float(eps), _stream())


def groupnorm_relu_fwd(x, gamma, beta, G=32, eps=1e-5, relu=True, out=None):
    N, H, W, C = x.shape
    HW = H * W
    y = torch.empty_like(x) if out is None else out
    mean = torch.empty((N, G), dtype=torch.float32, device=x.device)
    rstd = torch.empty((N, G), dtype=torch.float32, device=x.device)
    ws = workspace(load().utv2_groupnorm_workspace_floats(N, HW, C), x.device, "gn")
    call("utv2_groupnorm_relu_fwd", _p(x), _p(gamma), _p(beta), _p(y), _p(mean), _p(rstd), _p(ws), N, HW, C, G,
         float(eps), int(relu), _stream())
    return y, mean, rstd


def groupnorm_relu_bwd(dy, y, x, mean, rstd, gamma, dgamma, dbeta, G=32, relu=True, out=None):
    N, H, W, C = x.shape
    HW = H * W
    dx = torch.empty_like(x) if out is None else out
    ws = workspace(load().utv2_groupnorm_workspace_floats(N, HW, C), x.device, "gn")
    call("utv2_groupnorm_relu_bwd", _p(dy), _p(y), _p(x), _p(mean), _p(rstd), _p(gamma), _p(dx), _p(dgamma), _p(dbeta),
         _p(ws), N, HW, C, G, int(relu), _stream())
    return dx


def _iarr(vals):
    return (ctypes.c_int * len(vals))(*[int(v) for v in vals])


def _farr(vals):
    return (ctypes.c_float * len(vals))(*[float(v) for v in vals])


def fcos_targets(level_hw, strides, soi, gt_boxes, gt_classes, gt_valid, gt_std, num_classes, drop_empty, active=None,
                 center_radius=0.0, batch=None, img0=0):
    n_gt, MAXG = gt_classes.shape
    N = n_gt if batch is None else int(batch)
    L = sum(h * w for h, w in level_hw)
    P = N * L
    dev = gt_boxes.device
    labels = torch.empty(P, dtype=torch.int32, device=dev)
    reg = torch.empty((P, 4), dtype=torch.float32, device=dev)
    bv = torch.empty((P, 4), dtype=torch.float32, device=dev)
    gi = torch.empty(P, dtype=torch.int32, device=dev)
    H = _iarr([h for h, _ in level_hw])
    W = _iarr([w for _, w in level_hw])
    S = _iarr(strides)
    flat = []
    for lo, hi in soi:
        flat += [lo, hi]
    so = _farr(flat)
    call("utv2_fcos_targets_range", len(level_hw), ctypes.cast(H, c_p), ctypes.cast(W, c_p), ctypes.cast(S, c_p),
         ctypes.cast(so, c_p), N, MAXG, _p(gt_boxes), _p(gt_classes), _p(gt_valid), _p(gt_std), int(img0), n_gt, num_classes,
         int(drop_empty), float(center_radius), _p(active), _p(labels), _p(reg), _p(bv), _p(gi), _stream())
    return labels, reg, bv, gi


def sigmoid_focal_fwd(logits, labels, alpha, gamma):
    P, C = logits.shape
    out = torch.empty(1, dtype=torch.float32, device=logits.device)
    ws = workspace(4096, logits.device, "loss")
    call("utv2_sigmoid_focal_fwd", _p(logits), _p(labels), P, C, float(alpha), float(gamma), _p(out), _p(ws), _stream())
    return out


def sigmoid_focal_bwd(logits, labels, alpha, gamma, coef, out=None):
    P, C = logits.shape
    if out is None:
        out = torch.empty_like(logits)
    call("utv2_sigmoid_focal_bwd", _p(logits), _p(labels), P, C, float(alpha), float(gamma), _p(coef), _p(out), _stream())
    return out


def sigmoid_focal_bwd_acc(logits, labels, alpha, gamma, coef, gscale, out, accumulate):
    P, C = logits.shape
    call("utv2_sigmoid_focal_bwd_acc", _p(logits), _p(labels), P, C, float(alpha), float(gamma), _p(coef), _p(gscale), _p(out),
         int(bool(accumulate)), _stream())
    return out


def fcos_loc_terms_bwd_acc(labels, box, reg_targets, bvars, num_classes, reg_max, ts_better, ts_cert, coef8, gscale, out, accumulate, flags=0):
    P, BS = box.shape
    call("utv2_fcos_loc_terms_bwd_acc", _p(labels), _p(box), BS, _p(reg_targets), _p(bvars), P, num_classes, reg_max, float(ts_better),
         float(ts_cert), int(flags), _p(coef8), _p(gscale), _p(out), int(bool(accumulate)), _stream())
    return out


LT_QUALITY_IOU, LT_KLLOSS, LT_LOC_IOU, LT_LOC_LINEAR_IOU, LT_KL_WCTR = 1, 2, 1 << 2, 2 << 2, 16


def fcos_loc_terms_fwd(labels, box, reg_targets, bvars, num_classes, reg_max, ts_better, ts_cert, flags=0):
    P, BS = box.shape
    sums = torch.empty(8, dtype=torch.float32, device=box.device)
    ws = workspace(4096, box.device, "loss")
    call("utv2_fcos_loc_terms_fwd", _p(labels), _p(box), BS, _p(reg_targets), _p(bvars), P, num_classes, reg_max,
         float(ts_better), float(ts_cert), int(flags), _p(sums), _p(ws), _stream())
    return sums


def fcos_loss_combine(focal_sup, sums_sup, focal_cls, sums_cls, sums_reg, norm, world, flags, kl_weight, wmul, wdiv):
    dev = sums_sup.device
    rec = torch.empty(8, dtype=torch.float32, device=dev)
    coef = torch.empty(26, dtype=torch.float32, device=dev)
    call("utv2_fcos_loss_combine", _p(focal_sup), _p(sums_sup), _p(focal_cls), _p(sums_cls), _p(sums_reg), _p(norm), float(world), int(flags),
         float(kl_weight), ctypes.cast(_farr(wmul), c_p), ctypes.cast(_farr(wdiv), c_p), _p(rec), _p(coef), _stream())
    return rec, coef


def fcos_loc_terms_bwd(labels, box, reg_targets, bvars, num_classes, reg_max, ts_better, ts_cert, coef, out=None, flags=0):
    P, BS = box.shape
    if out is None:
        out = torch.empty_like(box)
    call("utv2_fcos_loc_terms_bwd", _p(labels), _p(box), BS, _p(reg_targets), _p(bvars), P, num_classes, reg_max,
         float(ts_better), float(ts_cert), int(flags), _p(coef), _p(out), _stream())
    return out


def fcos_rank_keys(logits, box, reg_max, N, HW, thr, method, out=None, row_stride=None):
    C = logits.shape[-1]
    BS = box.shape[-1]
    if out is None:
        out = torch.empty((N, HW * C), dtype=torch.int64, device=logits.device)
        row_stride = HW * C
    assert out.stride(1) == 1 and out.stride(0) == row_stride and out.shape[0] == N and out.shape[1] >= HW * C
    call("utv2_fcos_rank_keys", _p_any(logits), _p_any(box), BS, reg_max, N, HW, C, float(thr), method, c_p(out.data_ptr()),
         int(row_stride), _stream())
    return out


def topk_rows(keys_flat, row_off, rows, max_width, k):
    out = torch.empty((rows, k), dtype=torch.int64, device=keys_flat.device)
    nbytes = load().utv2_topk_rows_workspace_bytes(rows, int(k))
    ws = workspace((nbytes + 3) // 4, keys_flat.device, "topk")
    call("utv2_topk_rows_i64", _p(keys_flat), _p(row_off), rows, int(max_width), int(k), _p(out), _p(ws), _stream())
    return out


def fcos_decode(topkeys, logits, box, reg_max, N, HW, Wl, stride, level, method, slot0, outs):
    K = topkeys.shape[1]
    C = logits.shape[-1]
    BS = box.shape[-1]
    MAXC = outs["scores"].shape[1]
    call("utv2_fcos_decode", _p(topkeys), K, _p(logits), _p(box), BS, reg_max, N, HW, Wl, C, stride, level, method, MAXC,
         slot0, _p(outs["boxes"]), _p(outs["scores"]), _p(outs["classes"]), _p(outs["locations"]), _p(outs["centerness"]),
         _p(outs["cls_confid"]), _p(outs["reg_pred_std"]), _p(outs["fpn_levels"]), _p(outs["valid"]), _stream())


REG_CONT = 0


def fcos_loc_terms_cont_fwd(labels, box, reg_targets, bvars, num_classes, ts_better, ts_cert, flags=0):
    P, BS = box.shape
    sums = torch.empty(8, dtype=torch.float32, device=box.device)
    ws = workspace(4096, box.device, "loss")
    call("utv2_fcos_loc_terms_cont_fwd", _p(labels), _p(box), BS, _p(reg_targets), _p(bvars), P, num_classes, float(ts_better),
         float(ts_cert), int(flags), _p(sums), _p(ws), _stream())
    return sums


def fcos_loc_terms_cont_bwd(labels, box, reg_targets, bvars, num_classes, ts_better, ts_cert, coef, out=None, flags=0):
    P, BS = box.shape
    if out is None:
        out = torch.empty_like(box)
    call("utv2_fcos_loc_terms_cont_bwd", _p(labels), _p(box), BS, _p(reg_targets), _p(bvars), P, num_classes, float(ts_better),
         float(ts_cert), int(flags), _p(coef), _p(out), _stream())
    return out


def fcos_loc_terms_cont_bwd_acc(labels, box, reg_targets, bvars, num_classes, ts_better, ts_cert, coef8, gscale, out, accumulate, flags=0):
    P, BS = box.shape
    call("utv2_fcos_loc_terms_cont_bwd_acc", _p(labels), _p(box), BS, _p(reg_targets), _p(bvars), P, num_classes, float(ts_better),
         float(ts_cert), int(flags), _p(coef8), _p(gscale), _p(out), int(bool(accumulate)), _stream())
    return out


def fcos_decode_cont(topkeys, logits, box, N, HW, Wl, stride, level, method, slot0, outs):
    K = topkeys.shape[1]
    C = logits.shape[-1]
    BS = box.shape[-1]
    MAXC = outs["scores"].shape[1]
    call("utv2_fcos_decode_cont", _p(topkeys), K, _p(logits), _p(box), BS, N, HW, Wl, C, stride, level, method, MAXC, slot0,
         _p(outs["boxes"]), _p(outs["scores"]), _p(outs["classes"]), _p(outs["locations"]), _p(outs["centerness"]),
         _p(outs["cls_confid"]), _p(outs["reg_pred_std"]), _p(outs["fpn_levels"]), _p(outs["valid"]), _stream())


def scale_cols(y2d, ncols, s):
    rows, BS = y2d.shape
    call("utv2_scale_cols", _p(y2d), rows, BS, ncols, _p(s), _stream())


def _i64arr(vals):
    return (ctypes.c_int64 * len(vals))(*[int(v) for v in vals])


def scale_cols_ml(y2d, rows, ncols, scales):
    assert len(rows) == len(scales) <= 8 and all(rows[i][1] == rows[i + 1][0] for i in range(len(rows) - 1))
    r0 = _i64arr([r[0] for r in rows] + [rows[-1][1]])
    sp = _ptr_array(scales)
    call("utv2_scale_cols_ml", _p(y2d), len(rows), ctypes.cast(r0, c_p), y2d.shape[1], ncols, ctypes.cast(sp, c_p), _stream())


def scale_cols_bwd_ml(g2d, ypost2d, rows, ncols, scales, sgrads):
    assert len(rows) == len(scales) == len(sgrads) <= 8 and all(rows[i][1] == rows[i + 1][0] for i in range(len(rows) - 1))
    r0 = _i64arr([r[0] for r in rows] + [rows[-1][1]])
    sp, gp = _ptr_array(scales), _ptr_array(sgrads)
    ws = workspace(8 * 1024, g2d.device, "loss")
    call("utv2_scale_cols_bwd_ml", _p(g2d), _p(ypost2d), len(rows), ctypes.cast(r0, c_p), g2d.shape[1], ncols, ctypes.cast(sp, c_p),
         ctypes.cast(gp, c_p), _p(ws), _stream())


def scale_cols_bwd_ml_pad16(g2d, ypost2d, rows, ncols, scales, sgrads, cpad):
    assert len(rows) == len(scales) == len(sgrads) <= 8 and all(rows[i][1] == rows[i + 1][0] for i in range(len(rows) - 1))
    r0 = _i64arr([r[0] for r in rows] + [rows[-1][1]])
    sp, gp = _ptr_array(scales), _ptr_array(sgrads)
    ws = workspace(8 * 1024, g2d.device, "loss")
    out = torch.empty((g2d.shape[0], cpad), dtype=h16_dtype(), device=g2d.device)
    call("utv2_scale_cols_bwd_ml_pad16", _p(g2d), _p(ypost2d), len(rows), ctypes.cast(r0, c_p), g2d.shape[1], ncols, ctypes.cast(sp, c_p),
         ctypes.cast(gp, c_p), _p(ws), _p(out), int(cpad), _stream())
    return out


def scale_cols_bwd(g2d, ypost2d, ncols, s):
    rows, BS = g2d.shape
    dsum = torch.empty(1, dtype=torch.float32, device=g2d.device)
    ws = workspace(4096, g2d.device, "loss")
    call("utv2_scale_cols_bwd", _p(g2d), _p(ypost2d), rows, BS, ncols, _p(s), _p(dsum), _p(ws), _stream())
    return dsum


def nms_batched(boxes, scores, classes, valid, iou_thr, class_aware=True, post_topk=-1, max_out=128):
    N, M = scores.shape
    keep = torch.empty((N, max_out), dtype=torch.int32, device=boxes.device)
    cnt = torch.empty(N, dtype=torch.int32, device=boxes.device)
    nbytes = load().utv2_nms_workspace_bytes(N, M)
    ws = workspace((nbytes + 3) // 4, boxes.device, "nms")
    call("utv2_nms_batched", _p(boxes), _p(scores), _p(classes), _p(valid), N, M, float(iou_thr), int(class_aware),
         int(post_topk), max_out, _p(keep), _p(cnt), _p(ws), _stream())
    return keep, cnt


def box_iou(a, b):
    A, B = a.shape[0], b.shape[0]
    out = torch.empty((A, B), dtype=torch.float32, device=a.device)
    call("utv2_box_iou", _p(a), _p(b), A, B, _p(out), _stream())
    return out


def match_boxes(boxes, gt_boxes, gt_valid, want_gt_max=False):
    N, G = gt_valid.shape
    shared = boxes.dim() == 2
    P = boxes.shape[-2]
    dev = gt_boxes.device
# ... 794 lines not shown
```

### unbiased-teacher-v2_amd/ubteacher/ops.py

```python
import os

import torch

from . import hip

_HOOKS = {}
PRECISION = ["fp32"]


def set_precision(p):
    assert p in ("fp32", "bf16", "fp16")
    PRECISION[0] = p
    hip.set_h16("fp16" if p == "fp16" else "bf16")


def amp():
    return PRECISION[0] != "fp32"


def act_dtype():
    return hip.h16_dtype() if amp() else torch.float32


_VERSION = [0]
# ... 192 lines not shown
        self.scales = None
        rec = bytearray()
        self.nrec = 0
        for (layer, sc), o in zip(self.layers, offs):
            so = -1
            if sc is not None:
                if self.scales is None:
                    self.scales = torch.empty(0, dtype=torch.float32, device=dev).set_(sc.untyped_storage())
                assert sc.untyped_storage().data_ptr() == self.scales.untyped_storage().data_ptr()
                so = sc.storage_offset()
            G = layer.groups
            if G == 1:
                rec += struct.pack("<qqqiiiiii", layer.w.offset, o, so, layer.cout, layer.k, layer.k, layer.cin, layer.dgrad_cout(), 0)
                self.nrec += 1
            else:
                assert sc is None and layer.dgrad_cout() == layer.cout
                Kg = layer.cout // G
                for gi in range(G):
                    rec += struct.pack("<qqqiiiiii", layer.w.offset + gi * Kg * layer.kred, o + gi * layer.cin * layer.k * layer.k * Kg, -1,
                                       Kg, layer.k, layer.k, layer.cin, Kg, 0)
                    self.nrec += 1
        self.table = torch.frombuffer(rec, dtype=torch.uint8).clone().to(dev)
        self.views = [self.bank[o:o + l.dgrad_cout() * l.k * l.k * l.cin].view(l.groups * l.cin, l.k * l.k * l.dgrad_cout() // l.groups)
                      for (l, _), o in zip(self.layers, offs)]
        self.dirty = False
        self.single.clear()

    def refresh_ahead(self):
        cur = self._current()
        if (self.bank is None or self.dirty or self.version == cur or self.h16 != hip.H16[0] or os.environ.get("UTV2_FLIP_AHEAD", "1") == "0"
                or STEP_GRAPH[0]):
            return
        dev = self.store.flat.device
        if dev.type != "cuda":
            return
        side = self.__dict__.get("_side")
        if side is None:
            side = self._side = torch.cuda.Stream(dev)
        side.wait_stream(torch.cuda.current_stream(dev))
        with torch.cuda.stream(side):
            hip.weight_flip_transpose_bf16_batched(self.store.flat, self.scales, self.bank, self.table, self.nrec)
            self._ahead = torch.cuda.Event()
            self._ahead.record(side)
        self.version = cur

    def _join_ahead(self):
        ev = self.__dict__.pop("_ahead", None)
        if ev is not None:
            torch.cuda.current_stream(self.store.flat.device).wait_event(ev)

    def get(self, layer, scale):
        cur = self._current()
        if "_ahead" in self.__dict__:
            self._join_ahead()
        i = self.slot.get(id(layer))
        if i is None:
            self.slot[id(layer)] = len(self.layers)
            self.layers.append((layer, scale))
            self.dirty = True
        elif self.version == cur and not self.dirty:
            return self.views[i]
        elif self.version != cur and (i is not None):
            if self.dirty or self.bank is None or self.h16 != hip.H16[0]:
                self._rebuild()
            hip.weight_flip_transpose_bf16_batched(self.store.flat, self.scales, self.bank, self.table, self.nrec)
            self.version = cur
            return self.views[self.slot[id(layer)]]
        ent = self.single.get(id(layer))
        if ent is None or ent[0] != cur:
            if layer.groups > 1:
                Kg = layer.cout // layer.groups
                img = torch.cat([hip.weight_flip_transpose_bf16(layer.w.t[gi * Kg:(gi + 1) * Kg], Kg, layer.k, layer.k, layer.cin, None)
                                 for gi in range(layer.groups)])
            else:
                img = hip.weight_flip_transpose_bf16(layer.w.t, layer.cout, layer.k, layer.k, layer.cin, scale)
            if layer.dgrad_cout() != layer.cout:
                img = torch.nn.functional.pad(img.view(layer.cin, layer.k * layer.k, layer.cout), (0, layer.dgrad_cout() - layer.cout)) \
                    .reshape(layer.cin, -1).contiguous()
            ent = (cur, img)
            self.single[id(layer)] = ent
        return ent[1]


class Conv:

    def __init__(self, w, cin, cout, k, stride=1, pad=0, bias=None, bn=None, relu=False, trainable=True,
                 kred=None, colscale=None, out_fp32=False, groups=1):
        self.w = w
        self.cin, self.cout, self.k, self.stride, self.pad = cin, cout, k, stride, pad
        self.groups = groups
        self.gconv = groups > 1 and bn is not None
        assert groups == 1 or (colscale is None and cout % groups == 0)
        assert not self.gconv or (k == 3 and pad == 1 and stride in (1, 2) and cin * groups == cout and bias is None
                                  and cin % 4 == 0)
        self.bias = bias
        self.bn = bn
        self.relu = relu
        self.trainable = trainable
        self.kred = kred if kred is not None else k * k * cin
        self.colscale = colscale
        self.out_fp32 = out_fp32
        self.dgrad_pad_small = False
        self.premask_input = False
        self.bias_by_gn = False
        self.gn_cpg = 0
        self._gn_part = None
        self.gnb_src = None
        self.grad_premasked = False
        self._wt = None
        self._wt_version = -1

    def scale_shift(self):
        if self.bn is not None:
            return self.bn.scale, self.bn.shift
        return None, (self.bias.t if self.bias is not None else None)

    def wt(self):
        v = (_VERSION[0], self.w.store.version)
        if self._wt is None or self._wt_version != v:
            self._wt = hip.weight_flip_transpose(self.w.t, self.cout, self.k, self.k, self.cin)
            self._wt_version = v
        return self._wt

    def wt16(self, scale=None):
        bank = getattr(self.w.store, "_flipbank", None)
        if bank is None:
            bank = self.w.store._flipbank = FlipBank(self.w.store)
        return bank.get(self, scale)

    def dgrad_cout(self):
        if self.k == 3 and self.stride == 1 and self.cout % 32 and self.cout % 8 == 0 and (self.cout > 32 or self.dgrad_pad_small):
            return (self.cout + 31) // 32 * 32
        return self.cout

    def use_bf16(self):
        return amp() and self.cin % 8 == 0 and self.kred == self.k * self.k * self.cin

    def use_bf16_wgrad(self):
        return (amp() and self.cin % 8 == 0 and self.cout % 8 == 0 and self.k * self.k <= 16
                and self.kred == self.k * self.k * self.cin)

    def gn_stats_fused(self):
        return self.gn_cpg == 8 and self.cout % 8 == 0 and not self.relu and os.environ.get("UTV2_GN_STATS_FUSED", "1") != "0"

    def bias_grad_from_gn(self):
        return self.bias_by_gn and self.bias is not None and self.trainable and self.use_bf16_wgrad() and self.use_bf16_dgrad() \
            and os.environ.get("UTV2_GN_BIAS_GRAD", "1") != "0"

    def use_bf16_dgrad(self):
        return amp() and self.cout % 8 == 0

    def __call__(self, x, residual=None, out=None, colscale_handle=None, meta=None):
        if torch.is_grad_enabled() and self.trainable:
            return _ConvFn.apply(x, residual, hook(x.device), self, (out, getattr(x, "_utv2_fanin", None), getattr(x, "_utv2_pair", None)),
                                 colscale_handle, meta)
        return self._forward(x, residual, out, colscale_handle, meta)

    def gconv_weight(self):
        return self.w.store.bf16(self.w) if amp() else self.w.t

    def _forward(self, x, residual, out, cs, meta, relu_bits=None):
        sc, sh = self.scale_shift()
        if self.gconv:
            assert meta is None and residual is None and out is None and cs is None and relu_bits is None
            w = self.gconv_weight()
            if x.dtype != w.dtype:
                raise RuntimeError("grouped conv: %s activation with %s weights (layer cout=%d)" % (x.dtype, w.dtype, self.cout))
            return hip.gconv3x3_fwd(x.contiguous(), w, self.groups, self.stride, sc, sh, self.relu,
                                    out_dtype=torch.float32 if self.out_fp32 else x.dtype)
        b16 = self.use_bf16()
        w = self.w.store.bf16(self.w) if b16 else self.w.t
        kw = {}
        if b16:
            kw["out_dtype"] = out.dtype if out is not None else (torch.float32 if self.out_fp32 else hip.h16_dtype())
        else:
            assert x.dtype == torch.float32, "the fp32 conv kernels take fp32 activations (layer cin=%d)" % self.cin
        if not b16 and not x.is_contiguous():
            x = x.contiguous()
        if self.groups > 1:
            assert meta is not None and self.k > 1 and residual is None and out is None and cs is None
        if meta is not None and self.k > 1:
            assert self.stride == 1 and self.pad == (self.k - 1) // 2
            if b16:
                part = None
                if self.gn_stats_fused() and out is None and residual is None and kw["out_dtype"] == hip.h16_dtype() and self.cin % 32 == 0:
                    part = hip.gn_part_buffer(x.shape[0], self.cout, x.device)
                y = hip.conv2d_ml_fwd_bf16(x, w, meta.level_hw, meta.N, scale=sc, bias=sh, residual=residual, k=self.k, pad=self.pad,
                                           relu=self.relu, out=out, groups=self.groups, gn_part=part, **kw)
                self._gn_part = (y.data_ptr(), part) if part is not None else None
            elif self.groups > 1:
                Kg = self.cout // self.groups
                y = torch.cat([hip.conv2d_ml_fwd(x[:, gi * self.cin:(gi + 1) * self.cin].contiguous(), w[gi * Kg:(gi + 1) * Kg], meta.level_hw,
                                                 meta.N, scale=None, bias=None if sh is None else sh[gi * Kg:(gi + 1) * Kg], k=self.k,
                                                 pad=self.pad, relu=self.relu) for gi in range(self.groups)], dim=1)
            else:
                y = hip.conv2d_ml_fwd(x, w, meta.level_hw, meta.N, scale=sc, bias=sh, residual=residual, k=self.k, pad=self.pad,
                                      relu=self.relu, out=out, **kw)
        elif meta is not None:
            fn = hip.conv2d_fwd_bf16 if b16 else hip.conv2d_fwd
            y = fn(x.view(1, x.shape[0], 1, x.shape[1]), w, scale=sc, bias=sh,
                   residual=None if residual is None else residual.view(1, x.shape[0], 1, -1), relu=self.relu,
                   out=None if out is None else out.view(1, x.shape[0], 1, -1), **kw).view(x.shape[0], self.cout)
        else:
            fn = hip.conv2d_fwd_bf16 if b16 else hip.conv2d_fwd
            if relu_bits is not None:
                kw["relu_bits"] = relu_bits
            y = fn(x, w, scale=sc, bias=sh, residual=residual, stride=self.stride, pad=self.pad, relu=self.relu, kh=self.k,
                   kw=self.k, out=out, **kw)
        if cs is not None:
            assert y.dtype == torch.float32
            if meta is not None and _scale_ml_on() and y.is_contiguous():
                hip.scale_cols_ml(y, meta.rows, self.colscale, [h.t for h in cs])
            elif meta is not None:
                for l, h in enumerate(cs):
                    r0, r1 = meta.rows[l]
                    hip.scale_cols(y[r0:r1], self.colscale, h.t)
            else:
                hip.scale_cols(y.view(-1, self.cout), self.colscale, cs.t)
        return y


class _ConvFn(torch.autograd.Function):
    @staticmethod
    def forward(ctx, x, residual, hk, layer, out_holder, cs, meta):
        out = out_holder[0]
        y = layer._forward(x, residual, out, cs, meta)
        ctx.layer = layer
        ctx.cs = cs
        ctx.meta = meta
        ctx.has_res = residual is not None
        ctx.x_bits = _bits_of(x) if (layer.premask_input and meta is None) else None
        ctx.handoff = getattr(x, "_utv2_handoff", None) if (layer.premask_input and meta is None and grad_handoff_on()) else None
        if GRAD_SYNC[0] is not None:
            GRAD_SYNC[0].on_forward(_sync_handles(layer, cs))
        ctx.save_for_backward(x, y if (layer.relu or cs is not None) else None)
        ctx.xshape = tuple(x.shape)
        ctx.gnb = None
        src = layer.gnb_src
        if src is not None and src._gnb_fwd is not None:
            gf, src._gnb_fwd = src._gnb_fwd, None
            if gf[0] == x.data_ptr() and x.is_contiguous() and tuple(gf[1].shape) == tuple(x.shape) and residual is None:
                ctx.gnb = (src, gf[1], gf[2])
        ctx.fanin = out_holder[1] if len(out_holder) > 1 else None
        ctx.pair = out_holder[2] if len(out_holder) > 2 else None
        return y

    @staticmethod
    def backward(ctx, dy):
        layer = ctx.layer
        if layer.gconv:
            return _ConvFn._backward_grouped(ctx, dy)
        x, y = ctx.saved_tensors
        dy = dy.contiguous()
        if not x.is_contiguous() and not (layer.use_bf16_wgrad() and layer.use_bf16_dgrad()):
            x = x.contiguous()
        sc, _ = layer.scale_shift()
        meta = ctx.meta
        gp_ready = None
        if (ctx.cs is not None and meta is not None and _scale_ml_on() and y.is_contiguous() and dy.dtype == torch.float32
                and layer.k > 1 and ctx.needs_input_grad[0] and layer.use_bf16_dgrad() and layer.use_bf16_wgrad()
                and layer.dgrad_cout() != layer.cout and not layer.relu and sc is None and not ctx.has_res
                and os.environ.get("UTV2_SCALE_BWD_PAD16", "1") != "0"):
            gp_ready = hip.scale_cols_bwd_ml_pad16(dy, y, meta.rows, layer.colscale, [h.t for h in ctx.cs], [h.g for h in ctx.cs],
                                                   layer.dgrad_cout())
        elif ctx.cs is not None:
            g = dy.clone()
            if meta is not None and _scale_ml_on() and y.is_contiguous():
                hip.scale_cols_bwd_ml(g, y, meta.rows, layer.colscale, [h.t for h in ctx.cs], [h.g for h in ctx.cs])
            elif meta is not None:
                for l, h in enumerate(ctx.cs):
                    r0, r1 = meta.rows[l]
                    dsum = hip.scale_cols_bwd(g[r0:r1], y[r0:r1], layer.colscale, h.t)
                    h.g.add_(dsum / h.t.view(-1))
            else:
                dsum = hip.scale_cols_bwd(g.view(-1, layer.cout), y.view(-1, layer.cout), layer.colscale, ctx.cs.t)
                ctx.cs.g.add_(dsum / ctx.cs.t.view(-1))
            dy = g
        gres = None
        d16 = layer.use_bf16_dgrad()
        fold = sc is not None and d16 and layer.use_bf16_wgrad() and layer.bias is None
        wsc = sc if fold else None
        relu = layer.relu and not (layer.grad_premasked and premask_on())
        if fold:
            g = hip.relu_bwd_scale(dy, y, None) if relu else dy
            gres = g if ctx.has_res else None
        elif ctx.has_res:
            gm = hip.relu_bwd_scale(dy, y if relu else None, None) if relu else dy
            gres = gm
            g = hip.relu_bwd_scale(gm, None, sc) if sc is not None else gm
        else:
            if relu or sc is not None:
                g = hip.relu_bwd_scale(dy, y if relu else None, sc)
            else:
                g = dy
        dx = None
        bias_done = False
        if meta is not None and layer.k > 1:
            G = layer.groups
            Kg = layer.cout // G
            if ctx.needs_input_grad[0]:
                if d16:
                    gp = gp_ready if gp_ready is not None else (g if layer.dgrad_cout() == layer.cout else hip.pad_cols_bf16(g, layer.dgrad_cout()))
                    other = ctx.fanin.take() if ctx.fanin is not None else None
                    if other is not None and (other.dtype != x.dtype or tuple(other.shape) != tuple(x.shape)):
                        raise RuntimeError("FanIn: stored gradient does not match the conv input")
                    dest = ctx.pair[0].grad_half(ctx.pair[1], x) if (ctx.pair is not None and other is None) else None
                    wt = layer.wt16(wsc)
                    if (ctx.gnb is not None and other is None and dest is None and x.dtype == hip.h16_dtype()
                            and hip.gnb_eligible(gp, wt, layer.k, layer.k - 1 - layer.pad, G)):
                        src, gx, bits = ctx.gnb
                        part = hip.gnb_part_buffer(x.shape[0], x.shape[1], x.device)
                        dx = hip.conv2d_ml_fwd_bf16(gp, wt, meta.level_hw, meta.N, k=layer.k, pad=layer.k - 1 - layer.pad, out_dtype=x.dtype,
                                                    groups=G, gnb=(bits, gx, part))
                        src._gnb_bwd = (dx.data_ptr(), part)
                    else:
                        dx = hip.conv2d_ml_fwd_bf16(gp, wt, meta.level_hw, meta.N, k=layer.k, pad=layer.k - 1 - layer.pad,
                                                    residual=other, out_dtype=x.dtype, out=dest, groups=G)
                elif G > 1:
                    dx = torch.cat([hip.conv2d_ml_dgrad(g[:, gi * Kg:(gi + 1) * Kg].contiguous(),
                                                        hip.weight_flip_transpose(layer.w.t[gi * Kg:(gi + 1) * Kg], Kg, layer.k, layer.k, layer.cin),
                                                        meta.level_hw, meta.N, layer.k, layer.pad) for gi in range(G)], dim=1)
                else:
                    dx = hip.conv2d_ml_dgrad(g, layer.wt(), meta.level_hw, meta.N, layer.k, layer.pad)
            if layer.use_bf16_wgrad():
                gw = gp[:, :layer.cout] if (d16 and ctx.needs_input_grad[0] and gp is not g) else g
                _wgrad_launch(lambda: hip.conv2d_wgrad_bf16(
                    x, gw, layer.w.g, hip.rowinfo_ml(meta.N, meta.level_hw, layer.pad, layer.k, x.device), layer.cin, layer.k, layer.k,
                    accumulate=True, db=layer.bias.g if (layer.bias is not None and not layer.bias_grad_from_gn()) else None, rowscale=wsc,
                    groups=G, x_pitch=x.stride(0)), x, gw, key=layer)
                bias_done = True
            elif G > 1:
                for gi in range(G):
                    xg, gg = x[:, gi * layer.cin:(gi + 1) * layer.cin].contiguous(), g[:, gi * Kg:(gi + 1) * Kg].contiguous()
                    _wgrad_launch(lambda xg=xg, gg=gg, gi=gi: hip.conv2d_ml_wgrad(xg, gg, layer.w.g[gi * Kg:(gi + 1) * Kg], meta.level_hw, meta.N,
                                                                                   layer.k, layer.pad, accumulate=True), xg, gg, key=layer)
            else:
                _wgrad_launch(lambda: hip.conv2d_ml_wgrad(x, g, layer.w.g, meta.level_hw, meta.N, layer.k, layer.pad, accumulate=True), x, g, key=layer)
        else:
            x4 = x.view(1, x.shape[0], 1, x.shape[1]) if meta is not None else x
            g4 = g.view(1, g.shape[0], 1, g.shape[1]) if meta is not None else g
            if ctx.needs_input_grad[0]:
                pm = x4 if (layer.premask_input and premask_on()) else None
                if d16 and layer.k == 1 and layer.stride == 2 and layer.pad == 0:
                    dxc = hip.conv2d_fwd_bf16(g4, layer.wt16(wsc), out_dtype=x.dtype)
                    dx = hip.zero_interleave2x(dxc, x4.shape[1], x4.shape[2], mask=pm)
                elif (d16 and layer.k == 3 and layer.stride == 2 and layer.pad == 1 and g4.shape[-1] % 32 == 0
                      and x4.shape[0] * x4.shape[1] * x4.shape[2] <= 65536):
                    gd = hip.zero_interleave2x(g4.contiguous(), x4.shape[1], x4.shape[2])
                    dx = hip.conv2d_fwd_bf16(gd, layer.wt16(wsc), pad=1, kh=3, kw=3, out_dtype=x.dtype, mask=pm)
                elif d16:
                    gd = g4
                    if layer.dgrad_cout() != layer.cout:
                        gd = hip.pad_cols_bf16(g4.reshape(-1, layer.cout), layer.dgrad_cout()).view(g4.shape[:-1] + (layer.dgrad_cout(),))
                    pb = ctx.x_bits if (pm is not None and relu_bits_on() and x.dtype == hip.h16_dtype()) else None
                    BITS_STATS["reads"] += pb is not None
                    dx = hip.conv2d_dgrad_bf16(gd, layer.wt16(wsc), tuple(x4.shape), layer.stride, layer.pad, layer.k, layer.k,
                                               out_dtype=x.dtype, mask=None if pb is not None else pm, mask_bits=pb)
                else:
                    dx = hip.conv2d_dgrad(g4, layer.wt(), tuple(x4.shape), layer.stride, layer.pad, layer.k, layer.k)
                    if pm is not None:
                        dx = hip.relu_bwd_scale(dx, x4, None)
                if meta is not None:
                    dx = dx.view(x.shape)
                elif ctx.handoff is not None and pm is not None and dx.dtype == hip.h16_dtype() and ctx.handoff.park(dx):
                    dx = None
            if layer.use_bf16_wgrad():
                n_, h_, w_, _ = x4.shape
                ri = hip.rowinfo_nhwc(n_, h_, w_, g4.shape[1], g4.shape[2], layer.stride, layer.pad, layer.k, layer.k, x.device)
                _wgrad_launch(lambda: hip.conv2d_wgrad_bf16(
                    x4, g4.reshape(-1, layer.cout), layer.w.g, ri, layer.cin, layer.k, layer.k, accumulate=True,
                    db=layer.bias.g if (layer.bias is not None and not layer.bias_grad_from_gn()) else None, rowscale=wsc), x4, g4, key=layer)
                bias_done = True
            else:
                _wgrad_launch(lambda: hip.conv2d_wgrad(x4, g4, layer.w.g, layer.stride, layer.pad, layer.k, layer.k, accumulate=True), x4, g4, key=layer)
        if layer.bias is not None and not bias_done:
            _wgrad_launch(lambda: hip.colsum(g.view(-1, layer.cout), layer.bias.g, accumulate=True), g, key=layer)
        if GRAD_SYNC[0] is not None:
            GRAD_SYNC[0].on_backward_done(_sync_handles(layer, ctx.cs))
        return dx, gres, None, None, None, None, None

    @staticmethod
    def _backward_grouped(ctx, dy):
        layer = ctx.layer
        x, y = ctx.saved_tensors
        w = layer.gconv_weight()
        g = dy.contiguous()
        if g.dtype != w.dtype:
            g = g.to(w.dtype)
        relu = layer.relu and not (layer.grad_premasked and premask_on())
        if relu:
            g = hip.relu_bwd_scale(g, y if y.dtype == g.dtype else y.to(g.dtype), None)
        sc, _ = layer.scale_shift()
        dx = None
        if ctx.needs_input_grad[0]:
            pm = x if (layer.premask_input and premask_on()) else None
            dx = hip.gconv3x3_dgrad(g, w, layer.groups, layer.stride, tuple(x.shape), scale=sc, mask=pm, out_dtype=x.dtype)
        _wgrad_launch(lambda: hip.gconv3x3_wgrad(x, g, layer.w.g, layer.groups, layer.stride, scale=sc, accumulate=True), x, g, key=layer)
        if GRAD_SYNC[0] is not None:
            GRAD_SYNC[0].on_backward_done(_sync_handles(layer))
        return dx, None, None, None, None, None, None


def _wgrad16(layer, x4, g4):
    if layer.gconv:
        _wgrad_launch(lambda: hip.gconv3x3_wgrad(x4, g4, layer.w.g, layer.groups, layer.stride, scale=layer.bn.scale, accumulate=True),
                      x4, g4, key=layer)
        return
    n_, h_, w_, _ = x4.shape
    ri = hip.rowinfo_nhwc(n_, h_, w_, g4.shape[1], g4.shape[2], layer.stride, layer.pad, layer.k, layer.k, x4.device)
    _wgrad_launch(lambda: hip.conv2d_wgrad_bf16(x4, g4.reshape(-1, layer.cout), layer.w.g, ri, layer.cin, layer.k, layer.k, accumulate=True,
                                                rowscale=layer.bn.scale), x4, g4, key=layer)


def _dgrad16(layer, g4, in_shape, mask=None, residual=None, post_mask=None, mask_bits=None, post_mask_bits=None):
    if mask_bits is not None:
        mask = None
    if post_mask_bits is not None:
        post_mask = None
    if layer.gconv:
        assert post_mask is None and post_mask_bits is None and mask_bits is None
        return hip.gconv3x3_dgrad(g4, layer.gconv_weight(), layer.groups, layer.stride, tuple(in_shape), scale=layer.bn.scale, mask=mask,
                                  residual=residual, out_dtype=hip.h16_dtype())
    BITS_STATS["reads"] += (mask_bits is not None) + (post_mask_bits is not None)
    return hip.conv2d_dgrad_bf16(g4, layer.wt16(layer.bn.scale), tuple(in_shape), layer.stride, layer.pad, layer.k, layer.k,
                                 out_dtype=hip.h16_dtype(), mask=mask, residual=residual, post_mask=post_mask, mask_bits=mask_bits,
                                 post_mask_bits=post_mask_bits)


class GradHandoff:
    _live = []

    def __init__(self):
        self.grad = None
        self.closed = False
        if len(GradHandoff._live) >= 64:
            del GradHandoff._live[:32]
        GradHandoff._live.append(self)

    def park(self, g):
        if self.closed or self.grad is not None:
            return False
        self.grad = g
        return True

    def take(self):
        self.closed = True
        g, self.grad = self.grad, None
        return g


def grad_handoff_on():
    return premask_on() and os.environ.get("UTV2_GRAD_HANDOFF", "1") != "0"


def relu_bits_on():
    return os.environ.get("UTV2_RELU_BITS", "1") != "0"


BITS_STATS = {"planes": 0, "reads": 0}


def _bits_of(t):
    b = getattr(t, "_utv2_relu_bits", None)
    if b is not None and (b[0] != t.data_ptr() or b[1] != t._version):
        return None
    return None if b is None else b[2]


def premask_on():
    return os.environ.get("UTV2_PREMASK", "1") != "0"


class _BottleneckFn(torch.autograd.Function):
    @staticmethod
    def forward(ctx, x, hk, block):
        c1, c2, c3, cs = block.conv1, block.conv2, block.conv3, block.shortcut
        res = cs._forward(x, None, None, None, None) if cs is not None else x
        b1 = b2 = b3 = None
        if relu_bits_on() and all(c.relu and c.cout % 8 == 0 for c in (c1, c2, c3)):
            planes, (n_, h_, w_, _) = [], x.shape
            for c in (c1, c2, c3):
                h_, w_ = hip.conv_out_size(h_, c.k, c.stride, c.pad), hip.conv_out_size(w_, c.k, c.stride, c.pad)
                planes.append(hip.relu_bits_buffer((n_, h_, w_, c.cout), x.device))
            if c2.gconv:
                planes[0] = planes[1] = None
            b1, b2, b3 = planes
            BITS_STATS["planes"] += sum(b is not None for b in planes)
        y1 = c1._forward(x, None, None, None, None, relu_bits=b1)
        y2 = c2._forward(y1, None, None, None, None, relu_bits=b2)
        y3 = c3._forward(y2, res, None, None, None, relu_bits=b3)
        ctx.block = block
        ctx.handoff = None
        if ctx.needs_input_grad[0] and grad_handoff_on() and getattr(x, "_utv2_handoff", None) is None:
            ctx.handoff = x._utv2_handoff = GradHandoff()
        ctx.bits = (_bits_of(x), b1, b2)
        if b3 is not None:
            y3._utv2_relu_bits = (y3.data_ptr(), y3._version, b3)
        ctx.save_for_backward(x, y1, y2, y3)
        if GRAD_SYNC[0] is not None:
            for l in (c1, c2, c3, cs):
                if l is not None:
                    GRAD_SYNC[0].on_forward(_sync_handles(l))
        return y3

    @staticmethod
    def backward(ctx, dy):
        block = ctx.block
        c1, c2, c3, cs = block.conv1, block.conv2, block.conv3, block.shortcut
        x, y1, y2, y3 = ctx.saved_tensors
        pre = premask_on()
        if pre and block.grad_premasked:
            gm = dy.contiguous()
        else:
            gm = hip.relu_bwd_scale(dy.contiguous(), y3, None)
        pm = x if (pre and block.input_relu) else None
        bx, b1, b2 = ctx.bits
        if pm is None:
            bx = None
        _wgrad16(c3, y2, gm)
        g2 = _dgrad16(c3, gm, y2.shape, mask=y2, mask_bits=b2)
        _wgrad16(c2, y1, g2)
        g1 = _dgrad16(c2, g2, y1.shape, mask=y1, mask_bits=b1)
        _wgrad16(c1, x, g1)
        if cs is not None:
            _wgrad16(cs, x, gm)
        dx = None
        if ctx.needs_input_grad[0]:
            parked = ctx.handoff.take() if ctx.handoff is not None else None
            if parked is not None and (parked.dtype != hip.h16_dtype() or tuple(parked.shape) != tuple(x.shape)):
                raise RuntimeError("GradHandoff: parked gradient of another shape / type")
            if cs is None:
                dx = _dgrad16(c1, g1, x.shape, residual=gm, post_mask=pm, post_mask_bits=bx)
                if parked is not None:
                    dx = dx + parked
            elif c1.stride == 2:
                c = hip.conv2d_fwd_bf16(gm, cs.wt16(cs.bn.scale), out_dtype=hip.h16_dtype())
                c = hip.conv2d_fwd_bf16(g1, c1.wt16(c1.bn.scale), residual=c, out_dtype=hip.h16_dtype())
                dx = hip.zero_interleave2x(c, x.shape[1], x.shape[2], mask=pm if bx is None else None, mask_bits=bx if pm is not None else None,
                                           add=parked)
                BITS_STATS["reads"] += (bx is not None and pm is not None)
            elif cs.stride == 2:
                assert c1.stride == 1 and cs.k == 1 and cs.pad == 0
                c = hip.conv2d_fwd_bf16(gm, cs.wt16(cs.bn.scale), out_dtype=hip.h16_dtype())
                d = hip.zero_interleave2x(c, x.shape[1], x.shape[2], add=parked)
                dx = _dgrad16(c1, g1, x.shape, residual=d, post_mask=pm, post_mask_bits=bx)
            else:
                d = _dgrad16(cs, gm, x.shape, residual=parked)
                dx = _dgrad16(c1, g1, x.shape, residual=d, post_mask=pm, post_mask_bits=bx)
        if GRAD_SYNC[0] is not None:
            for l in (c3, c2, c1, cs):
                if l is not None:
                    GRAD_SYNC[0].on_backward_done(_sync_handles(l))
        return dx, None, None


def _fused_frozen_block_on():
    return os.environ.get("UTV2_FUSED_FROZEN_BLOCK", "1") != "0"


def bottleneck(block, x):
    convs = [c for c in (block.conv1, block.conv2, block.conv3, block.shortcut) if c is not None]
    fused = (amp() and torch.is_grad_enabled() and x.dtype == hip.h16_dtype()
             and all(c.trainable and c.bn is not None and c.bias is None
                     and (c.gconv or (c.use_bf16() and c.use_bf16_wgrad() and c.use_bf16_dgrad())) for c in convs)
             and block.conv1.stride in (1, 2) and block.conv1.k == 1 and block.conv3.k == 1
             and not (block.conv1.gconv or block.conv3.gconv)
             and (block.conv1.stride == 1 or block.conv2.stride == 1)
             and (block.shortcut is None or block.shortcut.stride == max(block.conv1.stride, block.conv2.stride)))
    if fused:
        return _BottleneckFn.apply(x, hook(x.device), block)
    if (amp() and x.dtype == hip.h16_dtype() and x.is_contiguous() and _fused_frozen_block_on()
            and (not torch.is_grad_enabled() or not any(c.trainable for c in convs)) and not x.requires_grad
            and all(c.stride == 1 for c in convs) and block.conv1.k == 1 and block.conv2.k == 3 and block.conv3.k == 1
            and (block.shortcut is None or block.shortcut.k == 1) and block.conv3.cout == 256
            and all(c.bn is not None and c.bias is None and c.use_bf16() for c in convs)
            and x.shape[1] * x.shape[2] * 256 < 2 ** 31
            and block.conv2.groups == 1 and block.conv1.cout <= 64
            and hip.bottleneck_supported(block.conv1.cin, block.conv1.cout, block.shortcut is not None)):
        st = block.conv1.w.store
        (s1, b1), (s2, b2), (s3, b3) = block.conv1.scale_shift(), block.conv2.scale_shift(), block.conv3.scale_shift()
        kw = {}
# ... 148 lines not shown
class _GNFn(torch.autograd.Function):
    @staticmethod
    def forward(ctx, x, hk, layer, meta):
        y, mean, rstd = layer._fwd(x, meta, for_backward=ctx.needs_input_grad[0])
        ctx.layer = layer
        ctx.meta = meta
        if GRAD_SYNC[0] is not None:
            GRAD_SYNC[0].on_forward(_sync_handles(layer))
        ctx.save_for_backward(x, y, mean, rstd)
        return y

    @staticmethod
    def backward(ctx, dy):
        layer, meta = ctx.layer, ctx.meta
        x, y, mean, rstd = ctx.saved_tensors
        dy = dy.contiguous()
        conv = layer.bias_conv
        cs = conv is not None and conv.bias_grad_from_gn()
        if meta is None:
            N, H, W, C = x.shape
            dx = hip.groupnorm_relu_seg_bwd(dy.view(-1, C), y.view(-1, C), x.view(-1, C), [H * W] * N, mean, rstd, layer.gamma.t,
                                            layer.gamma.g, layer.beta.g, layer.groups, layer.relu, beta=layer.beta.t, want_colsum=cs)
        else:
            gb, layer._gnb_bwd = layer._gnb_bwd, None
            if gb is not None and gb[0] == dy.data_ptr() and dy.dtype == hip.h16_dtype():
                dx = hip.groupnorm_seg_bwd_p64(dy, x, meta.seg_rows, mean, rstd, layer.gamma.t, layer.gamma.g, layer.beta.g, layer.groups,
                                               gb[1], want_colsum=cs)
                GNB_STATS["fused"] += 1
            else:
                dx = hip.groupnorm_relu_seg_bwd(dy, y, x, meta.seg_rows, mean, rstd, layer.gamma.t, layer.gamma.g, layer.beta.g,
                                                layer.groups, layer.relu, beta=layer.beta.t, want_colsum=cs)
        if cs:
            dx, part = dx
            _wgrad_launch(lambda: hip.colsum_partials(part, conv.bias.g, accumulate=True), part, key=conv)
        if meta is None:
            dx = dx.view(x.shape)
        if GRAD_SYNC[0] is not None:
            GRAD_SYNC[0].on_backward_done(_sync_handles(layer))
        return dx, None, None, None


class _UpAddFn(torch.autograd.Function):
    @staticmethod
    def forward(ctx, lateral, top):
        return hip.upsample2x_add(lateral, top)

    @staticmethod
    def backward(ctx, dy):
        dy = dy.contiguous()
        return dy, hip.downsample2x_sum(dy)


def upsample2x_add(lateral, top):
    if torch.is_grad_enabled() and (lateral.requires_grad or top.requires_grad):
        return _UpAddFn.apply(lateral, top)
    return hip.upsample2x_add(lateral, top)


class _ReLUFn(torch.autograd.Function):
    @staticmethod
    def forward(ctx, x):
        y = torch.relu(x)
        ctx.save_for_backward(y)
        return y

    @staticmethod
    def backward(ctx, dy):
        (y,) = ctx.saved_tensors
        return hip.relu_bwd_scale(dy.contiguous(), y, None)


def relu(x):
    return _ReLUFn.apply(x) if (torch.is_grad_enabled() and x.requires_grad) else torch.relu(x)


class _FocalSumFn(torch.autograd.Function):
    @staticmethod
    def forward(ctx, logits, labels, alpha, gamma):
        ctx.alpha, ctx.gamma = alpha, gamma
        ctx.save_for_backward(logits, labels)
        return hip.sigmoid_focal_fwd(logits, labels, alpha, gamma)

    @staticmethod
    def backward(ctx, gout):
        logits, labels = ctx.saved_tensors
        return hip.sigmoid_focal_bwd(logits, labels, ctx.alpha, ctx.gamma, gout.reshape(1).contiguous().float()), None, None, None


def focal_loss_sum(logits, labels, alpha, gamma):
    return _FocalSumFn.apply(logits, labels, alpha, gamma)


def _loc_fwd(labels, box, reg_targets, bvars, nc, reg_max, tsb, tsc, flags):
    if reg_max == hip.REG_CONT:
        return hip.fcos_loc_terms_cont_fwd(labels, box, reg_targets, bvars, nc, tsb, tsc, flags=flags)
    return hip.fcos_loc_terms_fwd(labels, box, reg_targets, bvars, nc, reg_max, tsb, tsc, flags=flags)


def _loc_bwd_acc(labels, box, reg_targets, bvars, nc, reg_max, tsb, tsc, coef8, gscale, out, accumulate, flags):
    if reg_max == hip.REG_CONT:
        return hip.fcos_loc_terms_cont_bwd_acc(labels, box, reg_targets, bvars, nc, tsb, tsc, coef8, gscale, out, accumulate, flags=flags)
    return hip.fcos_loc_terms_bwd_acc(labels, box, reg_targets, bvars, nc, reg_max, tsb, tsc, coef8, gscale, out, accumulate, flags=flags)


class _LocTermsFn(torch.autograd.Function):
    @staticmethod
    def forward(ctx, box, labels, reg_targets, bvars, args):
        ctx.args = args
        ctx.has_bv = bvars is not None
        ctx.save_for_backward(box, labels, reg_targets, bvars if bvars is not None else labels)
        nc, reg_max, tsb, tsc = args[:4]
        return _loc_fwd(labels, box, reg_targets, bvars, nc, reg_max, tsb, tsc, args[4] if len(args) > 4 else 0)

    @staticmethod
    def backward(ctx, gsums):
        box, labels, reg_targets, bv = ctx.saved_tensors
        nc, reg_max, tsb, tsc = ctx.args[:4]
        coef = torch.stack((gsums[2], gsums[3], gsums[4], gsums[6])).contiguous().float()
        flags = ctx.args[4] if len(ctx.args) > 4 else 0
        if reg_max == hip.REG_CONT:
            d = hip.fcos_loc_terms_cont_bwd(labels, box, reg_targets, bv if ctx.has_bv else None, nc, tsb, tsc, coef, flags=flags)
        else:
            d = hip.fcos_loc_terms_bwd(labels, box, reg_targets, bv if ctx.has_bv else None, nc, reg_max, tsb, tsc, coef, flags=flags)
        return d, None, None, None, None


class _FcosCombineFn(torch.autograd.Function):

    @staticmethod
    def forward(ctx, focal_sup, sums_sup, focal_cls, sums_cls, sums_reg, norm, world, flags, kl_weight, wmul, wdiv):
        rec, coef = hip.fcos_loss_combine(focal_sup.detach(), sums_sup.detach(), focal_cls.detach(), sums_cls.detach(), sums_reg.detach(),
                                          norm, world, flags, kl_weight, wmul, wdiv)
        ctx.save_for_backward(coef)
        ctx.mark_non_differentiable(rec)
        return rec[7].clone(), rec

    @staticmethod
    def backward(ctx, g, _):
        c = ctx.saved_tensors[0] * g
        return (c[0:1], c[1:9], c[9:10], c[10:18], c[18:26]) + (None,) * 6


def fcos_loss_combine(focal_sup, sums_sup, focal_cls, sums_cls, sums_reg, norm, world, flags, kl_weight, wmul, wdiv):
    return _FcosCombineFn.apply(focal_sup, sums_sup, focal_cls, sums_cls, sums_reg, norm, world, flags, kl_weight, wmul, wdiv)


class _FcosJointLossFn(torch.autograd.Function):

    @staticmethod
    def forward(ctx, logits, box, targets, consts, norm_fn):
        (lab_s, reg_s), (lab_c, reg_c), (lab_r, reg_r, bv_r) = targets
        alpha, gamma, nc, rm, flags_s, flags_p, tsb, tsc, world, cflags, klw, wmul, wdiv = consts
        lg, bx = logits.detach(), box.detach()
        focal_s = hip.sigmoid_focal_fwd(lg, lab_s, alpha, gamma)
        sums_s = _loc_fwd(lab_s, bx, reg_s, None, nc, rm, 0.0, 0.0, flags_s)
        focal_c = hip.sigmoid_focal_fwd(lg, lab_c, alpha, gamma)
        sums_c = _loc_fwd(lab_c, bx, reg_c, None, nc, rm, 0.0, 0.0, flags_p)
        sums_r = _loc_fwd(lab_r, bx, reg_r, bv_r, nc, rm, tsb, tsc, flags_p)
        norm = norm_fn(sums_s, sums_c, sums_r)
        rec, coef = hip.fcos_loss_combine(focal_s, sums_s, focal_c, sums_c, sums_r, norm, world, cflags, klw, wmul, wdiv)
        ctx.consts = consts
        ctx.has_bv = bv_r is not None
        ctx.save_for_backward(lg, bx, lab_s, reg_s, lab_c, reg_c, lab_r, reg_r, bv_r if bv_r is not None else lab_r, coef)
        ctx.mark_non_differentiable(rec)
        return rec[7].clone(), rec

    @staticmethod
    def backward(ctx, g, _):
        lg, bx, lab_s, reg_s, lab_c, reg_c, lab_r, reg_r, bv_r, coef = ctx.saved_tensors
        alpha, gamma, nc, rm, flags_s, flags_p, tsb, tsc = ctx.consts[:8]
        gs = g.reshape(1).contiguous().float()
        dlg, dbx = torch.empty_like(lg), torch.empty_like(bx)
        hip.sigmoid_focal_bwd_acc(lg, lab_s, alpha, gamma, coef[0:1], gs, dlg, False)
        hip.sigmoid_focal_bwd_acc(lg, lab_c, alpha, gamma, coef[9:10], gs, dlg, True)
        _loc_bwd_acc(lab_s, bx, reg_s, None, nc, rm, 0.0, 0.0, coef[1:9], gs, dbx, False, flags_s)
        _loc_bwd_acc(lab_c, bx, reg_c, None, nc, rm, 0.0, 0.0, coef[10:18], gs, dbx, True, flags_p)
        _loc_bwd_acc(lab_r, bx, reg_r, bv_r if ctx.has_bv else None, nc, rm, tsb, tsc, coef[18:26], gs, dbx, True, flags_p)
        return dlg, dbx, None, None, None


def fcos_joint_loss(logits, box, targets, consts, norm_fn):
    return _FcosJointLossFn.apply(logits, box, targets, consts, norm_fn)


class _RcnnCombineFn(torch.autograd.Function):

    @staticmethod
    def forward(ctx, rpn_sup, rpn_uns, focal_sup, focal_uns, box_sup, box_uns, tgt_sup, tgt_uns, consts):
        rec, coef = hip.rcnn_loss_combine(rpn_sup.detach(), rpn_uns.detach(), focal_sup.detach(), focal_uns.detach(), box_sup.detach(),
                                          box_uns.detach(), tgt_sup, tgt_uns, *consts)
        ctx.save_for_backward(coef)
        ctx.mark_non_differentiable(rec)
        return rec[8].clone(), rec

    @staticmethod
    def backward(ctx, g, _):
        c = ctx.saved_tensors[0] * g
        return (torch.stack((c[2], c[3])), torch.stack((c[6], c[7])), c[0:1], c[4:5], c[1:2], c[5:6], None, None, None)


def rcnn_loss_combine(rpn_sup, rpn_uns, focal_sup, focal_uns, box_sup, box_uns, tgt_sup, tgt_uns, consts):
    return _RcnnCombineFn.apply(rpn_sup, rpn_uns, focal_sup, focal_uns, box_sup, box_uns, tgt_sup, tgt_uns, consts)


def fcos_loc_terms(box, labels, reg_targets, bvars, args):
    return _LocTermsFn.apply(box, labels, reg_targets, bvars, args)


class FanIn:
    _live = []

    def __init__(self, meta, levels):
        self.meta, self.levels = meta, levels
        self.buf = None
        self.closed = False
        if len(FanIn._live) >= 64:
            del FanIn._live[:32]
        FanIn._live.append(self)

    def store(self, C, dtype, device):
        if self.closed or self.buf is not None:
            return None
        m = self.meta
        buf = torch.empty((m.P, C), dtype=dtype, device=device)
        outs = [m.alias_view(buf, l) for l in range(self.levels)]
        r0 = m.rows[self.levels][0] if self.levels < len(m.rows) else m.P
        if r0 < m.P:
            buf[r0:].zero_()
        self.buf = buf
        return buf, outs

    def take(self):
        self.closed = True
        b, self.buf = self.buf, None
        return b

    @staticmethod
    def check():
        live, FanIn._live = FanIn._live, []
        for f in live:
            if f.buf is not None:
                raise RuntimeError("FanIn: a RoIAlign gradient was stored but the RPN dgrad that adds it never ran")
        parked, GradHandoff._live = GradHandoff._live, []
        for h in parked:
            if h.grad is not None:
                raise RuntimeError("GradHandoff: a lateral's input gradient was parked but the block that adds it never ran")


def fanin_enabled():
    return amp() and os.environ.get("UTV2_FANIN", "1") != "0"


class _AssembleFn(torch.autograd.Function):

    @staticmethod
    def forward(ctx, big_holder, rows, *levels):
        ctx.rows = rows
        return big_holder[0].view(big_holder[0].shape)

    @staticmethod
    def backward(ctx, g):
        g = g.contiguous()
        return (None, None) + tuple(g[r0:r1].view(shape) for (r0, r1, shape) in ctx.rows)


def assemble(big, rows, levels):
    return _AssembleFn.apply((big,), rows, *levels)


class _RoIAlignFn(torch.autograd.Function):
    @staticmethod
    def forward(ctx, rois, roi_batch, roi_valid, cfg, *feats):
        scales, min_level, out_size, per_image, fanin, pooler, ratio = cfg
        ctx.cfg = cfg[:3]
        ctx.mode = dict(pooler=pooler, sampling_ratio=ratio)
        ctx.per_image = per_image
        ctx.fanin = fanin
        ctx.shapes = [tuple(f.shape) for f in feats]
        ctx.fdtype = feats[0].dtype
        y = hip.roi_align_fwd([f.detach() for f in feats], scales, min_level, rois, roi_batch, roi_valid, out_size, **ctx.mode)
        if pooler == "ROIPool":
            y, argmax = y
            ctx.save_for_backward(rois, roi_batch, roi_valid, argmax)
        else:
            ctx.save_for_backward(rois, roi_batch, roi_valid)
        return y

    @staticmethod
    def backward(ctx, dy):
        rois, roi_batch, roi_valid = ctx.saved_tensors[:3]
        mode = dict(ctx.mode, argmax=ctx.saved_tensors[3] if len(ctx.saved_tensors) > 3 else None)
        scales, min_level, out_size = ctx.cfg
        N, C = ctx.shapes[0][0], ctx.shapes[0][3]
        R = rois.shape[0]
        if ctx.per_image > 0 and R == N * ctx.per_image and C <= 256 and out_size <= 7:
            st = ctx.fanin.store(C, ctx.fdtype, dy.device) if (ctx.fanin is not None and ctx.fdtype == hip.h16_dtype()) else None
            if st is not None and [tuple(o.shape) for o in st[1]] == [tuple(x) for x in ctx.shapes]:
                hip.roi_align_bwd_tiled(ctx.shapes, ctx.fdtype, scales, min_level, rois, roi_valid, dy.contiguous(), ctx.per_image, outs=st[1],
                                        **mode)
                return (None, None, None, None) + (None,) * len(ctx.shapes)
            if st is not None:
                ctx.fanin.take(); ctx.fanin.closed = False
            dfeats = hip.roi_align_bwd_tiled(ctx.shapes, ctx.fdtype, scales, min_level, rois, roi_valid, dy.contiguous(), ctx.per_image, **mode)
            return (None, None, None, None) + tuple(dfeats)
        dfeats = [torch.zeros(s, dtype=torch.float32, device=dy.device) for s in ctx.shapes]
        hip.roi_align_bwd(dfeats, scales, min_level, rois, roi_batch, roi_valid, dy.contiguous(), **mode)
        if ctx.fdtype != torch.float32:
            dfeats = [d.to(ctx.fdtype) for d in dfeats]
        return (None, None, None, None) + tuple(dfeats)


def roi_align(feats, scales, min_level, rois, roi_batch, roi_valid, out_size, rois_per_image=0, fanin=None, pooler="ROIAlignV2",
              sampling_ratio=0):
    if torch.is_grad_enabled() and any(f.requires_grad for f in feats):
        return _RoIAlignFn.apply(rois, roi_batch, roi_valid,
                                 (tuple(scales), min_level, out_size, int(rois_per_image), fanin, pooler, int(sampling_ratio)), *feats)
    y = hip.roi_align_fwd(list(feats), scales, min_level, rois, roi_batch, roi_valid, out_size, pooler=pooler, sampling_ratio=sampling_ratio)
    return y[0] if pooler == "ROIPool" else y


class _SoftmaxFocalFn(torch.autograd.Function):
    @staticmethod
    def forward(ctx, logits, target, gamma):
        ctx.gamma = gamma
        ctx.save_for_backward(logits, target)
        return hip.softmax_focal_fwd(logits.contiguous(), target, gamma)

    @staticmethod
    def backward(ctx, g):
        logits, target = ctx.saved_tensors
        return hip.softmax_focal_bwd(logits.contiguous(), target, ctx.gamma, g.reshape(1).contiguous().float()), None, None


def softmax_focal_sum(logits, target, gamma):
    return _SoftmaxFocalFn.apply(logits, target, gamma)


class _Subsample2Fn(torch.autograd.Function):

    @staticmethod
    def forward(ctx, x, out_holder):
        ctx.shape = tuple(x.shape)
        out = out_holder[0]
        out.copy_(x[:, ::2, ::2, :])
        return out

    @staticmethod
    def backward(ctx, g):
        dx = torch.zeros(ctx.shape, dtype=g.dtype, device=g.device)
        dx[:, ::2, ::2, :] = g
        return dx, None


def subsample2_into(x, out):
    if torch.is_grad_enabled() and x.requires_grad:
        return _Subsample2Fn.apply(x, (out,))
    out.copy_(x[:, ::2, ::2, :])
    return out
```

Before: 345.4.

## Fuse FCOS focal and localization loss branches into joint kernels with bf16 gradient handoff

Replaces the separate per-branch focal loss launches (supervised and pseudo-label classification) with one joint kernel that reads the logits once and accumulates both sums. The three localization-loss branches are likewise fused into one forward and one backward kernel. The focal backward can also write a padded 16-bit gradient straight into the classification conv's dgrad input, handed over through a parked Grad16Handoff token. The aim is to cut repeated reads of logits and box tensors, the extra launches, and a later cast and pad of the gradient. The cost is a more complex autograd handoff that raises an error if the parked gradient is never consumed.

```diff
diff --git a/include/utv2.h b/include/utv2.h
--- a/include/utv2.h
+++ b/include/utv2.h
@@ -155,6 +155,18 @@
 int utv2_fcos_loc_terms_bwd_acc(const int* labels, const float* box, int box_stride, const float* reg_targets, const float* bvars,
                                 int64_t P, int num_classes, int reg_max, float ts_better, float ts_cert, int flags, const float* coef8,
                                 const float* gscale, float* dbox, int accumulate, utv2_stream_t stream);
+int utv2_sigmoid_focal_joint_fwd(const float* logits, const int* labels_a, const int* labels_b, int64_t P, int C, float alpha, float gamma,
+                                 float* loss_sums, float* ws, utv2_stream_t stream);
+int utv2_sigmoid_focal_joint_bwd_pad16(const float* logits, const int* labels_a, const int* labels_b, int64_t P, int C, float alpha,
+                                       float gamma, const float* coef_a, const float* coef_b, const float* gscale, void* out16, int cpad,
+                                       utv2_stream_t stream);
+int utv2_fcos_loc_terms_joint_fwd(const int* const* labels, const float* box, int box_stride, const float* const* reg_targets,
+                                  const float* const* bvars, int64_t P, int num_classes, int reg_max, const float* ts_better,
+                                  const float* ts_cert, const int* flags, float* sums, float* ws, utv2_stream_t stream);
+int utv2_fcos_loc_terms_joint_bwd(const int* const* labels, const float* box, int box_stride, const float* const* reg_targets,
+                                  const float* const* bvars, int64_t P, int num_classes, int reg_max, const float* ts_better,
+                                  const float* ts_cert, const int* flags, const float* const* coef8, const float* gscale, float* dbox,
+                                  utv2_stream_t stream);
 int utv2_fcos_loss_combine(const float* focal_sup, const float* sums_sup, const float* focal_cls, const float* sums_cls,
                            const float* sums_reg, const float* norm, float world, int flags, float kl_weight, const float* wmul_host,
                            const float* wdiv_host, float* rec, float* coef, utv2_stream_t stream);
diff --git a/unbiased-teacher-v2_amd/csrc/fcos.hip b/unbiased-teacher-v2_amd/csrc/fcos.hip
--- a/unbiased-teacher-v2_amd/csrc/fcos.hip
+++ b/unbiased-teacher-v2_amd/csrc/fcos.hip
@@ -195,6 +195,76 @@
   }
 }
 
+__global__ __launch_bounds__(256) void focal_joint_fwd_kernel(const float* __restrict__ logits, const int* __restrict__ labels_a,
+                                                            const int* __restrict__ labels_b, size_t P, int C, float alpha, float gamma,
+                                                            float* __restrict__ partial) {
+  __shared__ float red[4];
+  float acc_a = 0.f, acc_b = 0.f;
+  const unsigned C4 = (unsigned)C >> 2, total4 = (unsigned)(P * (size_t)C4);
+  for (unsigned i4 = blockIdx.x * blockDim.x + threadIdx.x; i4 < total4; i4 += gridDim.x * blockDim.x) {
+    const unsigned row = i4 / C4;
+    const int c = (int)(i4 - row * C4) * 4;
+    const int la = labels_a[row], lb = labels_b[row];
+    if (la < 0 && lb < 0) continue;
+    const f32x4 v = ((const f32x4*)logits)[i4];
+    if (la >= 0) {
+#pragma unroll
+      for (int e = 0; e < 4; ++e) acc_a += focal_term(v[e], la == c + e ? 1.f : 0.f, alpha, gamma, nullptr);
+    }
+    if (lb >= 0) {
+#pragma unroll
+      for (int e = 0; e < 4; ++e) acc_b += focal_term(v[e], lb == c + e ? 1.f : 0.f, alpha, gamma, nullptr);
+    }
+  }
+  const float sa = block_reduce_sum(acc_a, red);
+  const float sb = block_reduce_sum(acc_b, red);
+  if (threadIdx.x == 0) {
+    partial[2 * blockIdx.x] = sa;
+    partial[2 * blockIdx.x + 1] = sb;
+  }
+}
+
+__global__ __launch_bounds__(256) void focal_joint_bwd_pad16_kernel(const float* __restrict__ logits, const int* __restrict__ labels_a,
+                                                                  const int* __restrict__ labels_b, size_t P, int C, float alpha,
+                                                                  float gamma, const float* __restrict__ coef_a,
+                                                                  const float* __restrict__ coef_b, const float* __restrict__ gscale,
+                                                                  h16_t* __restrict__ out, int cpad) {
+  const float gs = gscale ? gscale[0] : 1.f;
+  const float ka = coef_a[0] * gs, kb = coef_b[0] * gs;
+  const unsigned C4 = (unsigned)C >> 2, qp = (unsigned)cpad >> 2, total = (unsigned)(P * (size_t)qp);
+  for (unsigned i = blockIdx.x * blockDim.x + threadIdx.x; i < total; i += gridDim.x * blockDim.x) {
+    const unsigned row = i / qp, c4 = i - row * qp;
+    f32x4 g = {0.f, 0.f, 0.f, 0.f};
+    if (c4 < C4) {
+      const int la = labels_a[row], lb = labels_b[row];
+      if (la >= 0 || lb >= 0) {
+        const int c = (int)c4 * 4;
+        const f32x4 v = ((const f32x4*)logits)[(size_t)row * C4 + c4];
+        if (la >= 0) {
+#pragma unroll
+          for (int e = 0; e < 4; ++e) {
+            float ge;
+            focal_term(v[e], la == c + e ? 1.f : 0.f, alpha, gamma, &ge);
+            g[e] += ge * ka;
+          }
+        }
+        if (lb >= 0) {
+#pragma unroll
+          for (int e = 0; e < 4; ++e) {
+            float ge;
+            focal_term(v[e], lb == c + e ? 1.f : 0.f, alpha, gamma, &ge);
+            g[e] += ge * kb;
+          }
+        }
+      }
+    }
+    bf16x4_t o;
+#pragma unroll
+    for (int e = 0; e < 4; ++e) o[e] = (h16_t)g[e];
+    ((bf16x4_t*)out)[i] = o;
+  }
+}
+
 __global__ __launch_bounds__(256) void sum_partials_kernel(const float* __restrict__ partial, int n, int ncols,
                                                            float* __restrict__ out) {
   __shared__ double red[256];
@@ -318,6 +388,56 @@
 #define LT_KL_WCTR 16
 
 template <int R1>
+__device__ __forceinline__ void loc_fwd_row(const float* __restrict__ row, const float* __restrict__ tg, const float* __restrict__ bv,
+                                            float ts_better, float ts_cert, int flags, float* acc) {
+  float d[4], t[4];
+  integral4<R1>(row, d, (float(*)[R1]) nullptr);
+#pragma unroll
+  for (int b = 0; b < 4; ++b) t[b] = tg[b];
+  float ctr_t = sqrtf((fminf(t[0], t[2]) / fmaxf(t[0], t[2])) * (fminf(t[1], t[3]) / fmaxf(t[1], t[3])));
+  float iou;
+  const float gl = giou_ltrb(d, t, &iou, nullptr, (flags >> LT_LOC_SHIFT) & 3);
+  if (flags & LT_QUALITY_IOU) ctr_t = iou;
+  float nll = 0.f;
+  const float* sp = row + 4 * R1;
+  if (flags & LT_KLLOSS) {
+#pragma unroll
+    for (int b = 0; b < 4; ++b) {
+      const float n = fabsf(d[b] - t[b]);
+      nll += expf(-sp[b]) * (n < 1.f ? 0.5f * n * n : n - 0.5f) + 0.5f * sp[b];
+    }
+    iou = (flags & LT_KL_WCTR) ? ctr_t : 1.f;
+  } else {
+#pragma unroll
+    for (int b = 0; b < 4; ++b) {
+      const float sg = 1.f / (1.f + expf(-sp[b]));
+      const float sq = sg * sg;
+      const float df = t[b] - d[b];
+      nll += (df * df) / (2.f * sq) + 0.5f * logf(sq);
+    }
+    nll += 2.f * logf(2.f * 3.14159265358979323846f);
+  }
+  const float c = row[4 * R1 + 4];
+  const float bce = fmaxf(c, 0.f) - c * ctr_t + log1pf(expf(-fabsf(c)));
+  acc[0] += 1.f;
+  acc[1] += ctr_t;
+  acc[2] += bce;
+  acc[3] += gl * ctr_t;
+  acc[4] += nll * iou;
+  if (bv) {
+#pragma unroll
+    for (int b = 0; b < 4; ++b) {
+      const float cs = 1.f - 1.f / (1.f + expf(-sp[b]));
+      const float ct = 1.f - 1.f / (1.f + expf(-bv[b]));
+      if (ct > ts_cert && ct > cs + ts_better) {
+        acc[5] += 1.f;
+        acc[6] += fabsf(d[b] - t[b]);
+      }
+    }
+  }
+}
+
+template <int R1>
 __global__ __launch_bounds__(128) void fcos_loc_fwd_kernel(const int* __restrict__ labels, const float* __restrict__ box, int BS,
                                                          const float* __restrict__ reg_targets, const float* __restrict__ bvars,
                                                          size_t P, int num_classes, float ts_better, float ts_cert, int flags,
@@ -331,58 +451,85 @@
   for (; i < P; i += stride) {
     const int lab = labels[i];
     if (lab < 0 || lab == num_classes) continue;
-    const float* row = box + i * BS;
-    float d[4], t[4];
-    integral4<R1>(row, d, (float(*)[R1]) nullptr);
-#pragma unroll
-    for (int b = 0; b < 4; ++b) t[b] = reg_targets[i * 4 + b];
-    float ctr_t = sqrtf((fminf(t[0], t[2]) / fmaxf(t[0], t[2])) * (fminf(t[1], t[3]) / fmaxf(t[1], t[3])));
-    float iou;
-    const float gl = giou_ltrb(d, t, &iou, nullptr, (flags >> LT_LOC_SHIFT) & 3);
-    if (flags & LT_QUALITY_IOU) ctr_t = iou;
-    float nll = 0.f;
-    const float* sp = row + 4 * R1;
-    if (flags & LT_KLLOSS) {
-#pragma unroll
-      for (int b = 0; b < 4; ++b) {
-        const float n = fabsf(d[b] - t[b]);
-        nll += expf(-sp[b]) * (n < 1.f ? 0.5f * n * n : n - 0.5f) + 0.5f * sp[b];
-      }
-      iou = (flags & LT_KL_WCTR) ? ctr_t : 1.f;
-    } else {
-#pragma unroll
-      for (int b = 0; b < 4; ++b) {
-        const float sg = 1.f / (1.f + expf(-sp[b]));
-        const float sq = sg * sg;
-        const float df = t[b] - d[b];
-        nll += (df * df) / (2.f * sq) + 0.5f * logf(sq);
-      }
-      nll += 2.f * logf(2.f * 3.14159265358979323846f);
-    }
-    const float c = row[4 * R1 + 4];
-    const float bce = fmaxf(c, 0.f) - c * ctr_t + log1pf(expf(-fabsf(c)));
-    acc[0] += 1.f;
-    acc[1] += ctr_t;
-    acc[2] += bce;
-    acc[3] += gl * ctr_t;
-    acc[4] += nll * iou;
-    if (bvars) {
-#pragma unroll
-      for (int b = 0; b < 4; ++b) {
-        const float cs = 1.f - 1.f / (1.f + expf(-sp[b]));
-        const float ct = 1.f - 1.f / (1.f + expf(-bvars[i * 4 + b]));
-        if (ct > ts_cert && ct > cs + ts_better) {
-          acc[5] += 1.f;
-          acc[6] += fabsf(d[b] - t[b]);
-        }
-      }
-    }
+    loc_fwd_row<R1>(box + i * BS, reg_targets + i * 4, bvars ? bvars + i * 4 : nullptr, ts_better, ts_cert, flags, acc);
   }
 #pragma unroll
   for (int k = 0; k < LT_NSUM; ++k) {
     const float s = block_reduce_sum(acc[k], red);
     if (threadIdx.x == 0) partial[(size_t)blockIdx.x * LT_NSUM + k] = s;
   }
+}
+
+template <int R1>
+__device__ __forceinline__ void loc_bwd_row(const float* __restrict__ row, float* grow, int BS, const float* __restrict__ tg,
+                                            const float* __restrict__ bv, float ts_better, float ts_cert, int flags, float c_bce,
+                                            float c_giou, float c_nll, float c_l1, int accumulate) {
+  double d[4], t[4], dl[4], prob[4][R1];
+  int jm[4];
+#pragma unroll
+  for (int b = 0; b < 4; ++b) {
+    float m = -INFINITY;
+#pragma unroll
+    for (int j = 0; j < R1; ++j) m = fmaxf(m, row[b * R1 + j]);
+    int q = 0;
+#pragma unroll
+    for (int j = R1 - 1; j >= 0; --j)
+      if (row[b * R1 + j] == m) q = j;
+    double s = 0.0;
+#pragma unroll
+    for (int j = 0; j < R1; ++j) { prob[b][j] = exp((double)row[b * R1 + j] - (double)m); s += prob[b][j]; }
+    double acc = 0.0;
+#pragma unroll
+    for (int j = 0; j < R1; ++j) { prob[b][j] /= s; acc += prob[b][j] * (double)(j - q); }
+    jm[b] = q; dl[b] = acc; d[b] = (double)q + acc;
+    t[b] = (double)tg[b];
+  }
+  double ctr_t = sqrt((fmin(t[0], t[2]) / fmax(t[0], t[2])) * (fmin(t[1], t[3]) / fmax(t[1], t[3])));
+  double iou, gg[4];
+  giou_ltrb_f64(d, t, &iou, gg, (flags >> LT_LOC_SHIFT) & 3);
+  if (flags & LT_QUALITY_IOU) ctr_t = iou;
+  const float* sp = row + 4 * R1;
+  double dd[4], ds[4];
+#pragma unroll
+  for (int b = 0; b < 4; ++b) {
+    const double sg = 1.0 / (1.0 + exp(-(double)sp[b]));
+    const double df = d[b] == t[b] ? 0.0 : (t[b] - (double)jm[b]) - dl[b];
+    if (flags & LT_KLLOSS) {
+      const double n = fabs(df), es = exp(-(double)sp[b]);
+      const double sgn = df < 0.0 ? 1.0 : (df > 0.0 ? -1.0 : 0.0);
+      const double wk = (flags & LT_KL_WCTR) ? ctr_t : 1.0;
+      dd[b] = (double)c_giou * ctr_t * gg[b] + (double)c_nll * wk * es * fmin(n, 1.0) * sgn;
+      ds[b] = (double)c_nll * wk * (0.5 - es * (n < 1.0 ? 0.5 * n * n : n - 0.5));
+    } else {
+      dd[b] = (double)c_giou * ctr_t * gg[b] + (double)c_nll * iou * (-df / (sg * sg));
+      ds[b] = (double)c_nll * iou * (1.0 - sg) * (1.0 - (df * df) / (sg * sg));
+    }
+    if (bv) {
+      const float cs = 1.f - 1.f / (1.f + expf(-sp[b]));
+      const float ct = 1.f - 1.f / (1.f + expf(-bv[b]));
+      if (ct > ts_cert && ct > cs + ts_better) dd[b] += (double)c_l1 * (d[b] > t[b] ? 1.0 : (d[b] < t[b] ? -1.0 : 0.0));
+    }
+  }
+  const double c = (double)row[4 * R1 + 4];
+  const float dctr = (float)((double)c_bce * (1.0 / (1.0 + exp(-c)) - ctr_t));
+  if (accumulate) {
+#pragma unroll
+    for (int b = 0; b < 4; ++b)
+#pragma unroll
+      for (int j = 0; j < R1; ++j) grow[b * R1 + j] += (float)(dd[b] * prob[b][j] * ((double)(j - jm[b]) - dl[b]));
+#pragma unroll
+    for (int b = 0; b < 4; ++b) grow[4 * R1 + b] += (float)ds[b];
+    grow[4 * R1 + 4] += dctr;
+    return;
+  }
+#pragma unroll
+  for (int b = 0; b < 4; ++b)
+#pragma unroll
+    for (int j = 0; j < R1; ++j) grow[b * R1 + j] = (float)(dd[b] * prob[b][j] * ((double)(j - jm[b]) - dl[b]));
+#pragma unroll
+  for (int b = 0; b < 4; ++b) grow[4 * R1 + b] = (float)ds[b];
+  grow[4 * R1 + 4] = dctr;
+  for (int k = 4 * R1 + 5; k < BS; ++k) grow[k] = 0.f;
 }
 
 template <int R1>
@@ -404,73 +551,74 @@
         for (int k = 0; k < BS; k += 4) *(f32x4*)(grow + k) = f32x4{0.f, 0.f, 0.f, 0.f};
       continue;
     }
-    const float* row = box + i * BS;
-    double d[4], t[4], dl[4], prob[4][R1];
-    int jm[4];
-#pragma unroll
-    for (int b = 0; b < 4; ++b) {
-      float m = -INFINITY;
-#pragma unroll
-      for (int j = 0; j < R1; ++j) m = fmaxf(m, row[b * R1 + j]);
-      int q = 0;
-#pragma unroll
-      for (int j = R1 - 1; j >= 0; --j)
-        if (row[b * R1 + j] == m) q = j;
-      double s = 0.0;
-#pragma unroll
-      for (int j = 0; j < R1; ++j) { prob[b][j] = exp((double)row[b * R1 + j] - (double)m); s += prob[b][j]; }
-      double acc = 0.0;
-#pragma unroll
-      for (int j = 0; j < R1; ++j) { prob[b][j] /= s; acc += prob[b][j] * (double)(j - q); }
-      jm[b] = q; dl[b] = acc; d[b] = (double)q + acc;
-      t[b] = (double)reg_targets[i * 4 + b];
-    }
-    double ctr_t = sqrt((fmin(t[0], t[2]) / fmax(t[0], t[2])) * (fmin(t[1], t[3]) / fmax(t[1], t[3])));
-    double iou, gg[4];
-    giou_ltrb_f64(d, t, &iou, gg, (flags >> LT_LOC_SHIFT) & 3);
-    if (flags & LT_QUALITY_IOU) ctr_t = iou;
-    const float* sp = row + 4 * R1;
-    double dd[4], ds[4];
-#pragma unroll
-    for (int b = 0; b < 4; ++b) {
-      const double sg = 1.0 / (1.0 + exp(-(double)sp[b]));
-      const double df = d[b] == t[b] ? 0.0 : (t[b] - (double)jm[b]) - dl[b];
-      if (flags & LT_KLLOSS) {
-        const double n = fabs(df), es = exp(-(double)sp[b]);
-        const double sgn = df < 0.0 ? 1.0 : (df > 0.0 ? -1.0 : 0.0);
-        const double wk = (flags & LT_KL_WCTR) ? ctr_t : 1.0;
-        dd[b] = (double)c_giou * ctr_t * gg[b] + (double)c_nll * wk * es * fmin(n, 1.0) * sgn;
-        ds[b] = (double)c_nll * wk * (0.5 - es * (n < 1.0 ? 0.5 * n * n : n - 0.5));
-      } else {
-        dd[b] = (double)c_giou * ctr_t * gg[b] + (double)c_nll * iou * (-df / (sg * sg));
-        ds[b] = (double)c_nll * iou * (1.0 - sg) * (1.0 - (df * df) / (sg * sg));
-      }
-      if (bvars) {
-        const float cs = 1.f - 1.f / (1.f + expf(-sp[b]));
-        const float ct = 1.f - 1.f / (1.f + expf(-bvars[i * 4 + b]));
-        if (ct > ts_cert && ct > cs + ts_better) dd[b] += (double)c_l1 * (d[b] > t[b] ? 1.0 : (d[b] < t[b] ? -1.0 : 0.0));
-      }
-    }
-    const double c = (double)row[4 * R1 + 4];
-    const float dctr = (float)((double)c_bce * (1.0 / (1.0 + exp(-c)) - ctr_t));
-    if (accumulate) {
-#pragma unroll
-      for (int b = 0; b < 4; ++b)
-#pragma unroll
-        for (int j = 0; j < R1; ++j) grow[b * R1 + j] += (float)(dd[b] * prob[b][j] * ((double)(j - jm[b]) - dl[b]));
-#pragma unroll
-      for (int b = 0; b < 4; ++b) grow[4 * R1 + b] += (float)ds[b];
-      grow[4 * R1 + 4] += dctr;
-      continue;
-    }
-#pragma unroll
-    for (int b = 0; b < 4; ++b)
-#pragma unroll
-      for (int j = 0; j < R1; ++j) grow[b * R1 + j] = (float)(dd[b] * prob[b][j] * ((double)(j - jm[b]) - dl[b]));
-#pragma unroll
-    for (int b = 0; b < 4; ++b) grow[4 * R1 + b] = (float)ds[b];
-    grow[4 * R1 + 4] = dctr;
-    for (int k = 4 * R1 + 5; k < BS; ++k) grow[k] = 0.f;
+    loc_bwd_row<R1>(box + i * BS, grow, BS, reg_targets + i * 4, bvars ? bvars + i * 4 : nullptr, ts_better, ts_cert, flags, c_bce, c_giou,
+                    c_nll, c_l1, accumulate);
+  }
+}
+
+#define LT_JOINT 3
+struct LocBranch {
+  const int* labels;
+  const float* reg_targets;
+  const float* bvars;
+  const float* coef8;
+  float ts_better, ts_cert;
+  int flags;
+};
+struct LocJoint {
+  LocBranch b[LT_JOINT];
+};
+
+template <int R1>
+__global__ __launch_bounds__(128) void fcos_loc_joint_fwd_kernel(LocJoint J, const float* __restrict__ box, int BS, size_t P,
+                                                               int num_classes, float* __restrict__ partial) {
+  __shared__ float red[2];
+  float acc[LT_JOINT][LT_NSUM];
+#pragma unroll
+  for (int q = 0; q < LT_JOINT; ++q)
+#pragma unroll
+    for (int k = 0; k < LT_NSUM; ++k) acc[q][k] = 0.f;
+  size_t i = (size_t)blockIdx.x * blockDim.x + threadIdx.x;
+  const size_t stride = (size_t)gridDim.x * blockDim.x;
+  for (; i < P; i += stride) {
+#pragma unroll
+    for (int q = 0; q < LT_JOINT; ++q) {
+      const int lab = J.b[q].labels[i];
+      if (lab < 0 || lab == num_classes) continue;
+      loc_fwd_row<R1>(box + i * BS, J.b[q].reg_targets + i * 4, J.b[q].bvars ? J.b[q].bvars + i * 4 : nullptr, J.b[q].ts_better,
+                      J.b[q].ts_cert, J.b[q].flags, acc[q]);
+    }
+  }
+#pragma unroll
+  for (int q = 0; q < LT_JOINT; ++q)
+#pragma unroll
+    for (int k = 0; k < LT_NSUM; ++k) {
+      const float s = block_reduce_sum(acc[q][k], red);
+      if (threadIdx.x == 0) partial[((size_t)blockIdx.x * LT_JOINT + q) * LT_NSUM + k] = s;
+    }
+}
+
+template <int R1>
+__global__ __launch_bounds__(128) void fcos_loc_joint_bwd_kernel(LocJoint J, const float* __restrict__ box, int BS, size_t P,
+                                                               int num_classes, const float* __restrict__ gscale,
+                                                               float* __restrict__ dbox) {
+  size_t i = (size_t)blockIdx.x * blockDim.x + threadIdx.x;
+  const size_t stride = (size_t)gridDim.x * blockDim.x;
+  const float gs = gscale ? gscale[0] : 1.f;
+  for (; i < P; i += stride) {
+    float* grow = dbox + i * BS;
+    const int l0 = J.b[0].labels[i];
+    const bool first = !(l0 < 0 || l0 == num_classes);
+    if (!first)
+      for (int k = 0; k < BS; k += 4) *(f32x4*)(grow + k) = f32x4{0.f, 0.f, 0.f, 0.f};
+#pragma nounroll
+    for (int q = 0; q < LT_JOINT; ++q) {
+      const int lab = q == 0 ? l0 : J.b[q].labels[i];
+      if (lab < 0 || lab == num_classes) continue;
+      const float* coef = J.b[q].coef8;
+      loc_bwd_row<R1>(box + i * BS, grow, BS, J.b[q].reg_targets + i * 4, J.b[q].bvars ? J.b[q].bvars + i * 4 : nullptr, J.b[q].ts_better,
+                      J.b[q].ts_cert, J.b[q].flags, coef[2] * gs, coef[3] * gs, coef[4] * gs, coef[6] * gs, q == 0 ? 0 : 1);
+    }
   }
 }
 
@@ -1008,6 +1156,67 @@
   return utv2_launch_status();
 }
 
+static bool loc_joint_fill(LocJoint& J, const int* const* labels, const float* const* reg_targets, const float* const* bvars,
+                           const float* const* coef8, const float* ts_better, const float* ts_cert, const int* flags) {
+  if (!labels || !reg_targets || !bvars || !ts_better || !ts_cert || !flags) return false;
+  for (int q = 0; q < LT_JOINT; ++q) {
+    if (!labels[q] || !reg_targets[q] || (coef8 && !coef8[q]) || flags[q] < 0 || flags[q] >= 32 || ((flags[q] >> LT_LOC_SHIFT) & 3) > 2) return false;
+    J.b[q].labels = labels[q]; J.b[q].reg_targets = reg_targets[q]; J.b[q].bvars = bvars[q]; J.b[q].coef8 = coef8 ? coef8[q] : nullptr;
+    J.b[q].ts_better = ts_better[q]; J.b[q].ts_cert = ts_cert[q]; J.b[q].flags = flags[q];
+  }
+  return true;
+}
+
+int utv2_sigmoid_focal_joint_fwd(const float* logits, const int* labels_a, const int* labels_b, int64_t P, int C, float alpha, float gamma,
+                                 float* loss_sums, float* ws, hipStream_t stream) {
+  if (!logits || !labels_a || !labels_b || !loss_sums || !ws || P < 0 || C < 4 || (C & 3) || (uint64_t)P * (uint64_t)C >= (1ull << 32) ||
+      ((uintptr_t)logits & 15))
+    return UTV2_EARG;
+  hipLaunchKernelGGL(focal_joint_fwd_kernel, dim3(FOCAL_BLOCKS), dim3(256), 0, stream, logits, labels_a, labels_b, (size_t)P, C, alpha, gamma,
+                     ws);
+  hipLaunchKernelGGL(sum_partials_kernel, dim3(2), dim3(256), 0, stream, (const float*)ws, FOCAL_BLOCKS, 2, loss_sums);
+  return utv2_launch_status();
+}
+
+int utv2_sigmoid_focal_joint_bwd_pad16(const float* logits, const int* labels_a, const int* labels_b, int64_t P, int C, float alpha,
+                                       float gamma, const float* coef_a, const float* coef_b, const float* gscale, void* out16, int cpad,
+                                       hipStream_t stream) {
+  if (!logits || !labels_a || !labels_b || !coef_a || !coef_b || !out16 || P < 0 || C < 4 || (C & 3) || cpad < C || (cpad & 3) ||
+      (uint64_t)P * (uint64_t)(cpad >> 2) >= (1ull << 32) || ((uintptr_t)logits & 15) || ((uintptr_t)out16 & 7))
+    return UTV2_EARG;
+  if (P == 0) return UTV2_OK;
+  hipLaunchKernelGGL(focal_joint_bwd_pad16_kernel, dim3(2048), dim3(256), 0, stream, logits, labels_a, labels_b, (size_t)P, C, alpha, gamma,
+                     coef_a, coef_b, gscale, (h16_t*)out16, cpad);
+  return utv2_launch_status();
+}
+
+int utv2_fcos_loc_terms_joint_fwd(const int* const* labels, const float* box, int box_stride, const float* const* reg_targets,
+                                  const float* const* bvars, int64_t P, int num_classes, int reg_max, const float* ts_better,
+                                  const float* ts_cert, const int* flags, float* sums, float* ws, hipStream_t stream) {
+  LocJoint J;
+  if (!box || !sums || !ws || reg_max != 16 || box_stride < 4 * 17 + 5 || (box_stride & 3) || P < 0 ||
+      !loc_joint_fill(J, labels, reg_targets, bvars, nullptr, ts_better, ts_cert, flags))
+    return UTV2_EARG;
+  hipLaunchKernelGGL((fcos_loc_joint_fwd_kernel<17>), dim3(LOC_BLOCKS), dim3(128), 0, stream, J, box, box_stride, (size_t)P, num_classes, ws);
+  hipLaunchKernelGGL(sum_partials_kernel, dim3(LT_JOINT * LT_NSUM), dim3(256), 0, stream, (const float*)ws, LOC_BLOCKS, LT_JOINT * LT_NSUM,
+                     sums);
+  return utv2_launch_status();
+}
+
+int utv2_fcos_loc_terms_joint_bwd(const int* const* labels, const float* box, int box_stride, const float* const* reg_targets,
+                                  const float* const* bvars, int64_t P, int num_classes, int reg_max, const float* ts_better,
+                                  const float* ts_cert, const int* flags, const float* const* coef8, const float* gscale, float* dbox,
+                                  hipStream_t stream) {
+  LocJoint J;
+  if (!box || !dbox || !coef8 || reg_max != 16 || box_stride < 4 * 17 + 5 || (box_stride & 3) || P < 0 || cdiv(P, 128) > 0x7fffffffll ||
+      ((uintptr_t)dbox & 15) || !loc_joint_fill(J, labels, reg_targets, bvars, coef8, ts_better, ts_cert, flags))
+    return UTV2_EARG;
+  if (P == 0) return UTV2_OK;
+  hipLaunchKernelGGL((fcos_loc_joint_bwd_kernel<17>), dim3((unsigned)cdiv(P, 128)), dim3(128), 0, stream, J, box, box_stride, (size_t)P,
+                     num_classes, gscale, dbox);
+  return utv2_launch_status();
+}
+
 int utv2_fcos_rank_keys(const float* logits, const float* box, int box_stride, int reg_max, int N, int HW, int C, float thr,
                         int method, long long* keys, int64_t key_row_stride, hipStream_t stream) {
   if (!logits || !box || !keys || method < 0 || method > 3 || key_row_stride < (int64_t)HW * C) return UTV2_EARG;
diff --git a/unbiased-teacher-v2_amd/ubteacher/hip.py b/unbiased-teacher-v2_amd/ubteacher/hip.py
--- a/unbiased-teacher-v2_amd/ubteacher/hip.py
+++ b/unbiased-teacher-v2_amd/ubteacher/hip.py
@@ -510,6 +510,59 @@
     return sums
 
 
+def focal_joint_supported(logits, cpad=None):
+    P, C = logits.shape
+    if logits.dtype != torch.float32 or C < 4 or C % 4 or P * C >= 1 << 32:
+        return False
+    return cpad is None or (cpad >= C and cpad % 4 == 0 and P * (cpad // 4) < 1 << 32)
+
+
+def sigmoid_focal_joint_fwd(logits, labels_a, labels_b, alpha, gamma):
+    P, C = logits.shape
+    out = torch.empty(2, dtype=torch.float32, device=logits.device)
+    ws = workspace(16384, logits.device, "loss")
+    call("utv2_sigmoid_focal_joint_fwd", _p(logits), _p(labels_a), _p(labels_b), P, C, float(alpha), float(gamma), _p(out), _p(ws), _stream())
+    return out
+
+
+def sigmoid_focal_joint_bwd_pad16(logits, labels_a, labels_b, alpha, gamma, coef_a, coef_b, gscale, cpad):
+    P, C = logits.shape
+    out = torch.empty((P, cpad), dtype=h16_dtype(), device=logits.device)
+    call("utv2_sigmoid_focal_joint_bwd_pad16", _p(logits), _p(labels_a), _p(labels_b), P, C, float(alpha), float(gamma), _p(coef_a),
+         _p(coef_b), _p(gscale), _p(out), int(cpad), _stream())
+    return out
+
+
+def _loc_joint_args(labels, reg_targets, bvars, ts_better, ts_cert, flags):
+    assert len(labels) == len(reg_targets) == len(bvars) == len(ts_better) == len(ts_cert) == len(flags) == 3
+    for t in list(labels) + list(reg_targets) + [b for b in bvars if b is not None]:
+        assert t.is_cuda and t.is_contiguous(), "HIP ops need contiguous CUDA tensors"
+    bv = (ctypes.c_void_p * 3)(*[None if b is None else b.data_ptr() for b in bvars])
+    return (_ptr_array(labels), _ptr_array(reg_targets), bv, _farr(ts_better), _farr(ts_cert), _iarr(flags))
+
+
+def fcos_loc_terms_joint_fwd(labels, box, reg_targets, bvars, num_classes, reg_max, ts_better, ts_cert, flags):
+    P, BS = box.shape
+    la, rt, bv, tb, tc, fl = _loc_joint_args(labels, reg_targets, bvars, ts_better, ts_cert, flags)
+    sums = torch.empty((3, 8), dtype=torch.float32, device=box.device)
+    ws = workspace(16384, box.device, "loss")
+    call("utv2_fcos_loc_terms_joint_fwd", ctypes.cast(la, c_p), _p(box), BS, ctypes.cast(rt, c_p), ctypes.cast(bv, c_p), P, num_classes,
+         reg_max, ctypes.cast(tb, c_p), ctypes.cast(tc, c_p), ctypes.cast(fl, c_p), _p(sums), _p(ws), _stream())
+    return sums
+
+
+def fcos_loc_terms_joint_bwd(labels, box, reg_targets, bvars, num_classes, reg_max, ts_better, ts_cert, flags, coef8, gscale, out=None):
+    P, BS = box.shape
+    la, rt, bv, tb, tc, fl = _loc_joint_args(labels, reg_targets, bvars, ts_better, ts_cert, flags)
+    assert len(coef8) == 3 and all(c.is_cuda and c.is_contiguous() for c in coef8)
+    cf = _ptr_array(coef8)
+    if out is None:
+        out = torch.empty_like(box)
+    call("utv2_fcos_loc_terms_joint_bwd", ctypes.cast(la, c_p), _p(box), BS, ctypes.cast(rt, c_p), ctypes.cast(bv, c_p), P, num_classes,
+         reg_max, ctypes.cast(tb, c_p), ctypes.cast(tc, c_p), ctypes.cast(fl, c_p), ctypes.cast(cf, c_p), _p(gscale), _p(out), _stream())
+    return out
+
+
 def fcos_loss_combine(focal_sup, sums_sup, focal_cls, sums_cls, sums_reg, norm, world, flags, kl_weight, wmul, wdiv):
     dev = sums_sup.device
     rec = torch.empty(8, dtype=torch.float32, device=dev)
diff --git a/unbiased-teacher-v2_amd/ubteacher/ops.py b/unbiased-teacher-v2_amd/ubteacher/ops.py
--- a/unbiased-teacher-v2_amd/ubteacher/ops.py
+++ b/unbiased-teacher-v2_amd/ubteacher/ops.py
@@ -368,9 +368,19 @@
 
     def __call__(self, x, residual=None, out=None, colscale_handle=None, meta=None):
         if torch.is_grad_enabled() and self.trainable:
-            return _ConvFn.apply(x, residual, hook(x.device), self, (out, getattr(x, "_utv2_fanin", None), getattr(x, "_utv2_pair", None)),
-                                 colscale_handle, meta)
+            g16 = Grad16Handoff(self.dgrad_cout()) if self.takes_grad16(x, residual, out, colscale_handle, meta) else None
+            y = _ConvFn.apply(x, residual, hook(x.device), self, (out, getattr(x, "_utv2_fanin", None), getattr(x, "_utv2_pair", None), g16),
+                              colscale_handle, meta)
+            if g16 is not None:
+                y._utv2_g16 = g16
+            return y
         return self._forward(x, residual, out, colscale_handle, meta)
+
+    def takes_grad16(self, x, residual, out, cs, meta):
+        return (meta is not None and self.k > 1 and not self.gconv and self.groups == 1 and residual is None and out is None and cs is None
+                and not self.relu and self.out_fp32 and x.requires_grad and self.use_bf16() and self.use_bf16_dgrad()
+                and self.use_bf16_wgrad() and self.dgrad_cout() != self.cout and self.scale_shift()[0] is None
+                and self.bias is not None and not self.bias_grad_from_gn())
 
     def gconv_weight(self):
         return self.w.store.bf16(self.w) if amp() else self.w.t
@@ -459,6 +469,7 @@
                 ctx.gnb = (src, gf[1], gf[2])
         ctx.fanin = out_holder[1] if len(out_holder) > 1 else None
         ctx.pair = out_holder[2] if len(out_holder) > 2 else None
+        ctx.g16 = out_holder[3] if len(out_holder) > 3 else None
         return y
 
     @staticmethod
@@ -467,12 +478,13 @@
         if layer.gconv:
             return _ConvFn._backward_grouped(ctx, dy)
         x, y = ctx.saved_tensors
-        dy = dy.contiguous()
+        gp_ready = ctx.g16.take(dy) if ctx.g16 is not None else None
+        if gp_ready is None:
+            dy = dy.contiguous()
         if not x.is_contiguous() and not (layer.use_bf16_wgrad() and layer.use_bf16_dgrad()):
             x = x.contiguous()
         sc, _ = layer.scale_shift()
         meta = ctx.meta
-        gp_ready = None
         if (ctx.cs is not None and meta is not None and _scale_ml_on() and y.is_contiguous() and dy.dtype == torch.float32
                 and layer.k > 1 and ctx.needs_input_grad[0] and layer.use_bf16_dgrad() and layer.use_bf16_wgrad()
                 and layer.dgrad_cout() != layer.cout and not layer.relu and sc is None and not ctx.has_res
@@ -643,6 +655,33 @@
                                  post_mask_bits=post_mask_bits)
 
 
+class Grad16Handoff:
+    _live = []
+
+    def __init__(self, cpad):
+        self.cpad = cpad
+        self.g16 = None
+        self.token = None
+
+    def park(self, g16, like, seed):
+        assert self.g16 is None and g16.shape[0] == like.shape[0] and g16.shape[1] == self.cpad and g16.dtype == hip.h16_dtype()
+        self.g16 = g16
+        self.token = seed.reshape(1, 1).expand(like.shape)
+        if len(Grad16Handoff._live) >= 64:
+            del Grad16Handoff._live[:32]
+        Grad16Handoff._live.append(self)
+        return self.token
+
+    def take(self, dy):
+        if self.g16 is None:
+            return None
+        tok = self.token
+        if dy is None or dy.data_ptr() != tok.data_ptr() or tuple(dy.shape) != tuple(tok.shape) or dy.stride() != tok.stride():
+            raise RuntimeError("Grad16Handoff: a 16-bit gradient was parked but the conv's backward received another tensor")
+        g, self.g16, self.token = self.g16, None, None
+        return g
+
+
 class GradHandoff:
     _live = []
 
@@ -1097,11 +1136,25 @@
         (lab_s, reg_s), (lab_c, reg_c), (lab_r, reg_r, bv_r) = targets
         alpha, gamma, nc, rm, flags_s, flags_p, tsb, tsc, world, cflags, klw, wmul, wdiv = consts
         lg, bx = logits.detach(), box.detach()
-        focal_s = hip.sigmoid_focal_fwd(lg, lab_s, alpha, gamma)
-        sums_s = _loc_fwd(lab_s, bx, reg_s, None, nc, rm, 0.0, 0.0, flags_s)
-        focal_c = hip.sigmoid_focal_fwd(lg, lab_c, alpha, gamma)
-        sums_c = _loc_fwd(lab_c, bx, reg_c, None, nc, rm, 0.0, 0.0, flags_p)
-        sums_r = _loc_fwd(lab_r, bx, reg_r, bv_r, nc, rm, tsb, tsc, flags_p)
+        joint = joint_loss_kernels_on()
+        ctx.joint_focal = joint and hip.focal_joint_supported(lg)
+        ctx.joint_loc = joint and rm != hip.REG_CONT
+        sink = getattr(logits, "_utv2_g16", None)
+        ctx.g16 = sink if (ctx.joint_focal and sink is not None and hip.focal_joint_supported(lg, sink.cpad)) else None
+        if ctx.joint_focal:
+            focal = hip.sigmoid_focal_joint_fwd(lg, lab_s, lab_c, alpha, gamma)
+            focal_s, focal_c = focal[0:1], focal[1:2]
+        else:
+            focal_s = hip.sigmoid_focal_fwd(lg, lab_s, alpha, gamma)
+            focal_c = hip.sigmoid_focal_fwd(lg, lab_c, alpha, gamma)
+        if ctx.joint_loc:
+            sums = hip.fcos_loc_terms_joint_fwd((lab_s, lab_c, lab_r), bx, (reg_s, reg_c, reg_r), (None, None, bv_r), nc, rm,
+                                                (0.0, 0.0, tsb), (0.0, 0.0, tsc), (flags_s, flags_p, flags_p))
+            sums_s, sums_c, sums_r = sums[0], sums[1], sums[2]
+        else:
+            sums_s = _loc_fwd(lab_s, bx, reg_s, None, nc, rm, 0.0, 0.0, flags_s)
+            sums_c = _loc_fwd(lab_c, bx, reg_c, None, nc, rm, 0.0, 0.0, flags_p)
+            sums_r = _loc_fwd(lab_r, bx, reg_r, bv_r, nc, rm, tsb, tsc, flags_p)
         norm = norm_fn(sums_s, sums_c, sums_r)
         rec, coef = hip.fcos_loss_combine(focal_s, sums_s, focal_c, sums_c, sums_r, norm, world, cflags, klw, wmul, wdiv)
         ctx.consts = consts
@@ -1115,13 +1168,26 @@
         lg, bx, lab_s, reg_s, lab_c, reg_c, lab_r, reg_r, bv_r, coef = ctx.saved_tensors
         alpha, gamma, nc, rm, flags_s, flags_p, tsb, tsc = ctx.consts[:8]
         gs = g.reshape(1).contiguous().float()
-        dlg, dbx = torch.empty_like(lg), torch.empty_like(bx)
-        hip.sigmoid_focal_bwd_acc(lg, lab_s, alpha, gamma, coef[0:1], gs, dlg, False)
-        hip.sigmoid_focal_bwd_acc(lg, lab_c, alpha, gamma, coef[9:10], gs, dlg, True)
-        _loc_bwd_acc(lab_s, bx, reg_s, None, nc, rm, 0.0, 0.0, coef[1:9], gs, dbx, False, flags_s)
-        _loc_bwd_acc(lab_c, bx, reg_c, None, nc, rm, 0.0, 0.0, coef[10:18], gs, dbx, True, flags_p)
-        _loc_bwd_acc(lab_r, bx, reg_r, bv_r if ctx.has_bv else None, nc, rm, tsb, tsc, coef[18:26], gs, dbx, True, flags_p)
+        if ctx.g16 is not None:
+            dlg = ctx.g16.park(hip.sigmoid_focal_joint_bwd_pad16(lg, lab_s, lab_c, alpha, gamma, coef[0:1], coef[9:10], gs, ctx.g16.cpad), lg, gs)
+        else:
+            dlg = torch.empty_like(lg)
+            hip.sigmoid_focal_bwd_acc(lg, lab_s, alpha, gamma, coef[0:1], gs, dlg, False)
+            hip.sigmoid_focal_bwd_acc(lg, lab_c, alpha, gamma, coef[9:10], gs, dlg, True)
+        dbx = torch.empty_like(bx)
+        if ctx.joint_loc:
+            hip.fcos_loc_terms_joint_bwd((lab_s, lab_c, lab_r), bx, (reg_s, reg_c, reg_r), (None, None, bv_r if ctx.has_bv else None), nc, rm,
+                                         (0.0, 0.0, tsb), (0.0, 0.0, tsc), (flags_s, flags_p, flags_p),
+                                         (coef[1:9], coef[10:18], coef[18:26]), gs, out=dbx)
+        else:
+            _loc_bwd_acc(lab_s, bx, reg_s, None, nc, rm, 0.0, 0.0, coef[1:9], gs, dbx, False, flags_s)
+            _loc_bwd_acc(lab_c, bx, reg_c, None, nc, rm, 0.0, 0.0, coef[10:18], gs, dbx, True, flags_p)
+            _loc_bwd_acc(lab_r, bx, reg_r, bv_r if ctx.has_bv else None, nc, rm, tsb, tsc, coef[18:26], gs, dbx, True, flags_p)
         return dlg, dbx, None, None, None
+
+
+def joint_loss_kernels_on():
+    return os.environ.get("UTV2_JOINT_LOSS_KERNELS", "1") != "0"
 
 
 def fcos_joint_loss(logits, box, targets, consts, norm_fn):
@@ -1190,6 +1256,10 @@
         for h in parked:
             if h.grad is not None:
                 raise RuntimeError("GradHandoff: a lateral's input gradient was parked but the block that adds it never ran")
+        parked, Grad16Handoff._live = Grad16Handoff._live, []
+        for h in parked:
+            if h.g16 is not None:
+                raise RuntimeError("Grad16Handoff: a 16-bit gradient was parked but the conv whose backward reads it never ran")
 
 
 def fanin_enabled():
```

Measured after the change: 345.4 (median of 2 runs). About the same (+0.0%).
